# AleoNet/snarkVM

Measured on AMD Instinct MI355X. Metric: BLS12-377 G1 MSM scalar-point pairs/sec (+ Fr NTT elements/sec in ntt_*), higher is better.
Workload: dtype u32 limbs (29-bit radix) modular integer arithmetic, Fq 377-bit / Fr 253-bit; 1 GPU; G1 Pippenger MSM 2^24 (BASELINE.json configs[1]), bases (i+1)G registered in HBM, uniform scalars in HBM; independent instance per GPU; scalars=uniform, lg_ntt=24, window_bits=auto, base_tables=12, table_bits=22, pipelined_batch=True

## Files before the change

include/snarkvm_hip.h:

```cpp
#ifndef SNARKVM_HIP_H
#define SNARKVM_HIP_H

#include <stddef.h>
#include <stdint.h>

#ifdef __cplusplus
extern "C" {
#endif

typedef struct {
    int32_t code;
    char *message;
} RustError;

enum NTTInputOutputOrder { NN = 0, NR = 1, RN = 2, RR = 3 };
enum NTTDirection { Forward = 0, Inverse = 1 };
enum NTTType { Standard = 0, Coset = 1 };


RustError snarkvm_ntt(void *inout, uint32_t lg_domain_size, enum NTTInputOutputOrder ntt_order,
                      enum NTTDirection ntt_direction, enum NTTType ntt_type);

RustError snarkvm_polymul(void *out, size_t pcount, const void *polynomials, const void *plens, size_t ecount,
                          const void *evaluations, const void *elens, uint32_t lg_domain_size);

RustError snarkvm_msm(void *out, const void *points_with_infinity, size_t npoints, const void *scalars,
                      size_t ffi_affine_sz);
RustError snarkvm_hip_set_base_cache(int tables);
RustError snarkvm_hip_set_base_cache_verified(int tables);
void snarkvm_hip_base_cache_stats(uint64_t *out, int reset);


int snarkvm_hip_device_count(void);
int snarkvm_hip_batch_lanes(size_t npoints);
RustError snarkvm_hip_set_devices(const int32_t *ids, size_t n);
RustError snarkvm_hip_set_device(int device);
int snarkvm_hip_num_devices(void);

RustError snarkvm_hip_malloc(void **d_ptr, size_t bytes, int device);
RustError snarkvm_hip_free(void *d_ptr);
RustError snarkvm_hip_memcpy_h2d(void *d_dst, const void *src, size_t bytes);
RustError snarkvm_hip_memcpy_d2h(void *dst, const void *d_src, size_t bytes);
RustError snarkvm_hip_memcpy_d2d(void *d_dst, const void *d_src, size_t bytes);
RustError snarkvm_hip_memset(void *d_dst, int value, size_t bytes);

RustError snarkvm_hip_ntt_device(void *d_inout, uint32_t lg_domain_size, int ntt_order, int ntt_direction,
                                 int ntt_type);
RustError snarkvm_hip_ntt_device_batch(void *const *d_inouts, size_t count, uint32_t lg_domain_size, int ntt_order,
                                       const int *ntt_directions, const int *ntt_types);

RustError snarkvm_hip_polymul_device(void *d_out, size_t pcount, const void *const *d_polys, const size_t *plens, size_t ecount,
                                     const void *const *d_evals, const size_t *elens, uint32_t lg_domain_size);

RustError snarkvm_hip_scope_begin(const void *d_any);
RustError snarkvm_hip_scope_end(void);
enum { SNARKVM_HIP_SCOPE_ASYNC_MSM = 1, SNARKVM_HIP_SCOPE_STABLE_INPUTS = 2, SNARKVM_HIP_SCOPE_MSM_IN_STREAM = 4 };
RustError snarkvm_hip_scope_begin_ex(const void *d_any, uint32_t flags);
RustError snarkvm_hip_scope_collect(const void *out);
RustError snarkvm_hip_scope_set_flags(uint32_t flags);
void *snarkvm_hip_scope_stream(void);

typedef struct snarkvm_hip_bases snarkvm_hip_bases_t;
RustError snarkvm_hip_register_bases(snarkvm_hip_bases_t **handle, const void *points, size_t npoints,
                                     size_t ffi_affine_sz, int on_device);
RustError snarkvm_hip_register_bases_tables(snarkvm_hip_bases_t **handle, const void *points, size_t npoints,
                                            size_t ffi_affine_sz, int on_device, int tables);
RustError snarkvm_hip_register_bases_windowed(snarkvm_hip_bases_t **handle, const void *points, size_t npoints,
                                              size_t ffi_affine_sz, int on_device, int tables, int window_bits);
void snarkvm_hip_free_bases(snarkvm_hip_bases_t *handle);

RustError snarkvm_hip_register_bases_serialized(snarkvm_hip_bases_t **handle, const void *bytes, size_t npoints,
                                                int compressed, int validate, int tables);
RustError snarkvm_hip_g1_deserialize(void *out_affine, const void *bytes, size_t n, int compressed, int validate);
RustError snarkvm_hip_g1_serialize(void *out_bytes, const void *affine, size_t n, size_t ffi_affine_sz, int compressed);

RustError snarkvm_hip_g2_deserialize(void *out_affine, const void *bytes, size_t n, int validate);
RustError snarkvm_hip_g2_serialize(void *out_bytes, const void *affine, size_t n, size_t ffi_affine_sz);
RustError snarkvm_hip_g2_deserialize_compressed(void *out_affine, const void *bytes, size_t n, int validate);
RustError snarkvm_hip_g2_serialize_compressed(void *out_bytes, const void *affine, size_t n, size_t ffi_affine_sz);

RustError snarkvm_hip_msm_registered(void *out, const snarkvm_hip_bases_t *handle, size_t offset, size_t npoints,
                                     const void *scalars, int scalars_on_device, int window_bits);

RustError snarkvm_hip_msm_registered_ex(void *out, const snarkvm_hip_bases_t *handle, size_t off0, size_t n0,
                                        size_t off1, size_t n1, const void *scalars, int scalars_on_device,
                                        int scalars_montgomery, int window_bits);

RustError snarkvm_hip_msm_registered_batch(void *outs, const snarkvm_hip_bases_t *handle, size_t count,
                                           const size_t *offsets, const size_t *npoints, const void *const *scalars,
                                           int scalars_on_device, int scalars_montgomery, int window_bits);

RustError snarkvm_hip_msm_registered_batch_ex(void *outs, const snarkvm_hip_bases_t *handle, size_t count, const size_t *off0,
                                              const size_t *n0, const size_t *off1, const size_t *n1,
                                              const void *const *scalars, int scalars_on_device, int scalars_montgomery,
                                              int window_bits);

RustError snarkvm_hip_g1_sum(void *out, const void *in_projective, size_t n);

RustError snarkvm_hip_g1_to_affine(void *out_affine, const void *in_projective, size_t n);

RustError snarkvm_hip_msm_g2(void *out, const void *points_with_infinity, size_t npoints, const void *scalars,
                             size_t ffi_affine_sz);

typedef struct snarkvm_hip_bases_g2 snarkvm_hip_bases_g2_t;
RustError snarkvm_hip_register_bases_g2(snarkvm_hip_bases_g2_t **handle, const void *points, size_t npoints,
                                        size_t ffi_affine_sz, int tables, int window_bits);
void snarkvm_hip_free_bases_g2(snarkvm_hip_bases_g2_t *handle);
RustError snarkvm_hip_msm_g2_registered(void *out, const snarkvm_hip_bases_g2_t *handle, size_t offset, size_t npoints,
                                        const void *scalars, int scalars_on_device, int window_bits);
RustError snarkvm_hip_msm_g2_registered_batch(void *outs, const snarkvm_hip_bases_g2_t *handle, size_t count,
                                              const size_t *offsets, const size_t *npoints, const void *const *scalars,
                                              int scalars_on_device, int window_bits);

RustError snarkvm_hip_g1_fixed_base_msm(void *out_projective, const void *g_affine, const void *scalars, size_t n);
RustError snarkvm_hip_g1_group_ntt(void *inout_projective, uint32_t lg_domain_size, int inverse);

RustError snarkvm_hip_fr_mul_device(void *d_out, const void *d_a, const void *d_b, size_t n);
RustError snarkvm_hip_fr_convert_device(void *d_out, const void *d_in, size_t n, int to_bigint);

RustError snarkvm_hip_fr_vec_op(int op, void *out, const void *a, const void *b, const void *c, const void *scalar,
                                size_t n, int on_device);
RustError snarkvm_hip_fr_divide_by_linear(void *quotient, void *remainder, const void *poly, size_t n,
                                          const void *point, int on_device);
RustError snarkvm_hip_fr_batch_inversion_and_mul(void *inout, size_t n, const void *coeff, int on_device);
RustError snarkvm_hip_fr_distribute_powers(void *inout, size_t n, const void *g, const void *c, int on_device);
RustError snarkvm_hip_fr_lagrange_coefficients(void *out, uint32_t lg_domain_size, const void *tau, int on_device);
RustError snarkvm_hip_fr_divide_by_vanishing(void *quotient, void *remainder, const void *poly, size_t len,
                                             size_t domain_size, int on_device);
RustError snarkvm_hip_fr_mul_by_vanishing(void *out, const void *poly, size_t len, size_t domain_size, int on_device);

RustError snarkvm_hip_fr_lincomb(void *out, size_t n_out, size_t count, const void *const *polys, const size_t *lens, const void *coeffs,
                                 int on_device);

enum { SNARKVM_HIP_FR_REDUCE_SUM = 0, SNARKVM_HIP_FR_REDUCE_DOT = 1 };
RustError snarkvm_hip_fr_reduce(int op, void *result, const void *a, const void *b, size_t n, int on_device);
RustError snarkvm_hip_fr_reduce_strided(int op, void *results, const void *a, const void *b, size_t n, size_t count, size_t stride,
                                        int b_shared);
RustError snarkvm_hip_fr_support(uint64_t *out3, const void *v, size_t n, int on_device);
RustError snarkvm_hip_fr_support_strided(uint64_t *out, const void *v, size_t n, size_t count, size_t stride);

typedef struct snarkvm_hip_fr_matrix snarkvm_hip_fr_matrix_t;
RustError snarkvm_hip_fr_matrix_register(snarkvm_hip_fr_matrix_t **handle, size_t rows, size_t cols, const uint64_t *row_ptr, const uint32_t *col_idx,
                                         const void *vals);
void snarkvm_hip_fr_matrix_free(snarkvm_hip_fr_matrix_t *handle);
RustError snarkvm_hip_fr_spmv(void *y, size_t n_out, const snarkvm_hip_fr_matrix_t *handle, const void *x, size_t count, size_t stride_x, size_t stride_y,
                              int on_device);

RustError snarkvm_hip_fr_vec_op_strided(int op, void *out, const void *a, const void *b, const void *c, const void *scalar,
                                        size_t n, size_t count, size_t stride);
RustError snarkvm_hip_fr_divide_by_linear_strided(void *quotients, void *remainders, const void *polys, size_t n,
                                                  const void *point, size_t count, size_t stride);
RustError snarkvm_hip_fr_divide_by_vanishing_strided(void *quotients, void *remainders, const void *polys, size_t len,
// ... 47 lines not shown
```

rust/snarkvm-algorithms-hip/src/sys.rs:

```rust
#![allow(non_camel_case_types, non_snake_case, clippy::too_many_arguments, clippy::missing_safety_doc)]
use super::{Error, NTTDirection, NTTInputOutputOrder, NTTType};
use core::ffi::{c_char, c_void};

#[repr(C)]
pub struct snarkvm_hip_bases_t {
    _private: [u8; 0],
}
#[repr(C)]
pub struct snarkvm_hip_bases_g2_t {
    _private: [u8; 0],
}
#[repr(C)]
pub struct snarkvm_hip_fr_matrix_t {
    _private: [u8; 0],
}

pub const SNARKVM_HIP_SCOPE_ASYNC_MSM: u32 = 1;
pub const SNARKVM_HIP_SCOPE_STABLE_INPUTS: u32 = 2;
pub const SNARKVM_HIP_SCOPE_MSM_IN_STREAM: u32 = 4;
pub const SNARKVM_HIP_FR_REDUCE_SUM: u32 = 0;
pub const SNARKVM_HIP_FR_REDUCE_DOT: u32 = 1;

extern "C" {
    pub fn snarkvm_ntt(inout: *mut c_void, lg_domain_size: u32, ntt_order: NTTInputOutputOrder, ntt_direction: NTTDirection, ntt_type: NTTType) -> Error;
    pub fn snarkvm_polymul(out: *mut c_void, pcount: usize, polynomials: *const c_void, plens: *const c_void, ecount: usize, evaluations: *const c_void, elens: *const c_void, lg_domain_size: u32) -> Error;
    pub fn snarkvm_msm(out: *mut c_void, points_with_infinity: *const c_void, npoints: usize, scalars: *const c_void, ffi_affine_sz: usize) -> Error;
    pub fn snarkvm_hip_set_base_cache(tables: i32) -> Error;
    pub fn snarkvm_hip_set_base_cache_verified(tables: i32) -> Error;
    pub fn snarkvm_hip_base_cache_stats(out: *mut u64, reset: i32);
    pub fn snarkvm_hip_device_count() -> i32;
    pub fn snarkvm_hip_batch_lanes(npoints: usize) -> i32;
    pub fn snarkvm_hip_set_devices(ids: *const i32, n: usize) -> Error;
    pub fn snarkvm_hip_set_device(device: i32) -> Error;
    pub fn snarkvm_hip_num_devices() -> i32;
    pub fn snarkvm_hip_malloc(d_ptr: *mut *mut c_void, bytes: usize, device: i32) -> Error;
    pub fn snarkvm_hip_free(d_ptr: *mut c_void) -> Error;
    pub fn snarkvm_hip_memcpy_h2d(d_dst: *mut c_void, src: *const c_void, bytes: usize) -> Error;
    pub fn snarkvm_hip_memcpy_d2h(dst: *mut c_void, d_src: *const c_void, bytes: usize) -> Error;
    pub fn snarkvm_hip_memcpy_d2d(d_dst: *mut c_void, d_src: *const c_void, bytes: usize) -> Error;
    pub fn snarkvm_hip_memset(d_dst: *mut c_void, value: i32, bytes: usize) -> Error;
    pub fn snarkvm_hip_ntt_device(d_inout: *mut c_void, lg_domain_size: u32, ntt_order: i32, ntt_direction: i32, ntt_type: i32) -> Error;
    pub fn snarkvm_hip_ntt_device_batch(d_inouts: *const *mut c_void, count: usize, lg_domain_size: u32, ntt_order: i32, ntt_directions: *const i32, ntt_types: *const i32) -> Error;
    pub fn snarkvm_hip_polymul_device(d_out: *mut c_void, pcount: usize, d_polys: *const *const c_void, plens: *const usize, ecount: usize, d_evals: *const *const c_void, elens: *const usize, lg_domain_size: u32) -> Error;
    pub fn snarkvm_hip_scope_begin(d_any: *const c_void) -> Error;
    pub fn snarkvm_hip_scope_end() -> Error;
    pub fn snarkvm_hip_scope_begin_ex(d_any: *const c_void, flags: u32) -> Error;
    pub fn snarkvm_hip_scope_collect(out: *const c_void) -> Error;
    pub fn snarkvm_hip_scope_set_flags(flags: u32) -> Error;
    pub fn snarkvm_hip_scope_stream() -> *mut c_void;
    pub fn snarkvm_hip_register_bases(handle: *mut *mut snarkvm_hip_bases_t, points: *const c_void, npoints: usize, ffi_affine_sz: usize, on_device: i32) -> Error;
    pub fn snarkvm_hip_register_bases_tables(handle: *mut *mut snarkvm_hip_bases_t, points: *const c_void, npoints: usize, ffi_affine_sz: usize, on_device: i32, tables: i32) -> Error;
    pub fn snarkvm_hip_register_bases_windowed(handle: *mut *mut snarkvm_hip_bases_t, points: *const c_void, npoints: usize, ffi_affine_sz: usize, on_device: i32, tables: i32, window_bits: i32) -> Error;
    pub fn snarkvm_hip_free_bases(handle: *mut snarkvm_hip_bases_t);
    pub fn snarkvm_hip_register_bases_serialized(handle: *mut *mut snarkvm_hip_bases_t, bytes: *const c_void, npoints: usize, compressed: i32, validate: i32, tables: i32) -> Error;
    pub fn snarkvm_hip_g1_deserialize(out_affine: *mut c_void, bytes: *const c_void, n: usize, compressed: i32, validate: i32) -> Error;
    pub fn snarkvm_hip_g1_serialize(out_bytes: *mut c_void, affine: *const c_void, n: usize, ffi_affine_sz: usize, compressed: i32) -> Error;
    pub fn snarkvm_hip_g2_deserialize(out_affine: *mut c_void, bytes: *const c_void, n: usize, validate: i32) -> Error;
    pub fn snarkvm_hip_g2_serialize(out_bytes: *mut c_void, affine: *const c_void, n: usize, ffi_affine_sz: usize) -> Error;
    pub fn snarkvm_hip_g2_deserialize_compressed(out_affine: *mut c_void, bytes: *const c_void, n: usize, validate: i32) -> Error;
    pub fn snarkvm_hip_g2_serialize_compressed(out_bytes: *mut c_void, affine: *const c_void, n: usize, ffi_affine_sz: usize) -> Error;
    pub fn snarkvm_hip_msm_registered(out: *mut c_void, handle: *const snarkvm_hip_bases_t, offset: usize, npoints: usize, scalars: *const c_void, scalars_on_device: i32, window_bits: i32) -> Error;
    pub fn snarkvm_hip_msm_registered_ex(out: *mut c_void, handle: *const snarkvm_hip_bases_t, off0: usize, n0: usize, off1: usize, n1: usize, scalars: *const c_void, scalars_on_device: i32, scalars_montgomery: i32, window_bits: i32) -> Error;
    pub fn snarkvm_hip_msm_registered_batch(outs: *mut c_void, handle: *const snarkvm_hip_bases_t, count: usize, offsets: *const usize, npoints: *const usize, scalars: *const *const c_void, scalars_on_device: i32, scalars_montgomery: i32, window_bits: i32) -> Error;
    pub fn snarkvm_hip_msm_registered_batch_ex(outs: *mut c_void, handle: *const snarkvm_hip_bases_t, count: usize, off0: *const usize, n0: *const usize, off1: *const usize, n1: *const usize, scalars: *const *const c_void, scalars_on_device: i32, scalars_montgomery: i32, window_bits: i32) -> Error;
    pub fn snarkvm_hip_g1_sum(out: *mut c_void, in_projective: *const c_void, n: usize) -> Error;
    pub fn snarkvm_hip_g1_to_affine(out_affine: *mut c_void, in_projective: *const c_void, n: usize) -> Error;
    pub fn snarkvm_hip_msm_g2(out: *mut c_void, points_with_infinity: *const c_void, npoints: usize, scalars: *const c_void, ffi_affine_sz: usize) -> Error;
    pub fn snarkvm_hip_register_bases_g2(handle: *mut *mut snarkvm_hip_bases_g2_t, points: *const c_void, npoints: usize, ffi_affine_sz: usize, tables: i32, window_bits: i32) -> Error;
    pub fn snarkvm_hip_free_bases_g2(handle: *mut snarkvm_hip_bases_g2_t);
    pub fn snarkvm_hip_msm_g2_registered(out: *mut c_void, handle: *const snarkvm_hip_bases_g2_t, offset: usize, npoints: usize, scalars: *const c_void, scalars_on_device: i32, window_bits: i32) -> Error;
    pub fn snarkvm_hip_msm_g2_registered_batch(outs: *mut c_void, handle: *const snarkvm_hip_bases_g2_t, count: usize, offsets: *const usize, npoints: *const usize, scalars: *const *const c_void, scalars_on_device: i32, window_bits: i32) -> Error;
    pub fn snarkvm_hip_g1_fixed_base_msm(out_projective: *mut c_void, g_affine: *const c_void, scalars: *const c_void, n: usize) -> Error;
    pub fn snarkvm_hip_g1_group_ntt(inout_projective: *mut c_void, lg_domain_size: u32, inverse: i32) -> Error;
    pub fn snarkvm_hip_fr_mul_device(d_out: *mut c_void, d_a: *const c_void, d_b: *const c_void, n: usize) -> Error;
    pub fn snarkvm_hip_fr_convert_device(d_out: *mut c_void, d_in: *const c_void, n: usize, to_bigint: i32) -> Error;
    pub fn snarkvm_hip_fr_vec_op(op: i32, out: *mut c_void, a: *const c_void, b: *const c_void, c: *const c_void, scalar: *const c_void, n: usize, on_device: i32) -> Error;
    pub fn snarkvm_hip_fr_divide_by_linear(quotient: *mut c_void, remainder: *mut c_void, poly: *const c_void, n: usize, point: *const c_void, on_device: i32) -> Error;
    pub fn snarkvm_hip_fr_batch_inversion_and_mul(inout: *mut c_void, n: usize, coeff: *const c_void, on_device: i32) -> Error;
    pub fn snarkvm_hip_fr_distribute_powers(inout: *mut c_void, n: usize, g: *const c_void, c: *const c_void, on_device: i32) -> Error;
    pub fn snarkvm_hip_fr_lagrange_coefficients(out: *mut c_void, lg_domain_size: u32, tau: *const c_void, on_device: i32) -> Error;
    pub fn snarkvm_hip_fr_divide_by_vanishing(quotient: *mut c_void, remainder: *mut c_void, poly: *const c_void, len: usize, domain_size: usize, on_device: i32) -> Error;
    pub fn snarkvm_hip_fr_mul_by_vanishing(out: *mut c_void, poly: *const c_void, len: usize, domain_size: usize, on_device: i32) -> Error;
    pub fn snarkvm_hip_fr_lincomb(out: *mut c_void, n_out: usize, count: usize, polys: *const *const c_void, lens: *const usize, coeffs: *const c_void, on_device: i32) -> Error;
    pub fn snarkvm_hip_fr_reduce(op: i32, result: *mut c_void, a: *const c_void, b: *const c_void, n: usize, on_device: i32) -> Error;
    pub fn snarkvm_hip_fr_reduce_strided(op: i32, results: *mut c_void, a: *const c_void, b: *const c_void, n: usize, count: usize, stride: usize, b_shared: i32) -> Error;
    pub fn snarkvm_hip_fr_support(out3: *mut u64, v: *const c_void, n: usize, on_device: i32) -> Error;
    pub fn snarkvm_hip_fr_support_strided(out: *mut u64, v: *const c_void, n: usize, count: usize, stride: usize) -> Error;
    pub fn snarkvm_hip_fr_matrix_register(handle: *mut *mut snarkvm_hip_fr_matrix_t, rows: usize, cols: usize, row_ptr: *const u64, col_idx: *const u32, vals: *const c_void) -> Error;
    pub fn snarkvm_hip_fr_matrix_free(handle: *mut snarkvm_hip_fr_matrix_t);
    pub fn snarkvm_hip_fr_spmv(y: *mut c_void, n_out: usize, handle: *const snarkvm_hip_fr_matrix_t, x: *const c_void, count: usize, stride_x: usize, stride_y: usize, on_device: i32) -> Error;
    pub fn snarkvm_hip_fr_vec_op_strided(op: i32, out: *mut c_void, a: *const c_void, b: *const c_void, c: *const c_void, scalar: *const c_void, n: usize, count: usize, stride: usize) -> Error;
    pub fn snarkvm_hip_fr_divide_by_linear_strided(quotients: *mut c_void, remainders: *mut c_void, polys: *const c_void, n: usize, point: *const c_void, count: usize, stride: usize) -> Error;
    pub fn snarkvm_hip_fr_divide_by_vanishing_strided(quotients: *mut c_void, remainders: *mut c_void, polys: *const c_void, len: usize, domain_size: usize, count: usize, stride: usize) -> Error;
    pub fn snarkvm_hip_g1_generate_bases_device(d_out: *mut c_void, start: u64, npoints: usize) -> Error;
    pub fn snarkvm_hip_set_profiling(enabled: i32);
    pub fn snarkvm_hip_get_phase_count() -> i32;
    pub fn snarkvm_hip_get_phase_name(i: i32) -> *const c_char;
    pub fn snarkvm_hip_get_phase_ms(i: i32) -> f64;
    pub fn snarkvm_hip_coalescer_stats(out: *mut u64, reset: i32);
    pub fn snarkvm_hip_alloc_stats(out: *mut u64, reset: i32);
    pub fn snarkvm_hip_synchronize() -> Error;
    pub fn snarkvm_hip_selftest_field(field: i32, op: i32, a: *const c_void, b: *const c_void, out: *mut c_void, n: usize) -> i32;
    pub fn snarkvm_hip_selftest_g1_msm_naive(points_with_infinity: *const c_void, npoints: usize, ffi_affine_sz: usize, scalars: *const c_void, out: *mut c_void) -> i32;
    pub fn snarkvm_hip_selftest_msm_plan(n: usize, window_bits: i32, tables: i32, table_bits: i32, out: *mut u32) -> i32;
    pub fn snarkvm_hip_selftest_g1_finish(planes_projective: *const c_void, pos: *const i32, n: usize, out: *mut c_void) -> i32;
    pub fn snarkvm_hip_selftest_fq_lazy(seed: u64, iters: i32) -> i32;
    pub fn snarkvm_hip_selftest_g1_lazy_tail(seed: u64, iters: i32) -> i32;
    pub fn snarkvm_hip_selftest_fq2_pair(points: *const c_void, npoints: usize, seed: u64, iters: i32) -> i32;
    pub fn snarkvm_hip_selftest_g2_hex(points: *const c_void, npoints: usize, seed: u64, iters: i32) -> i32;
    pub fn snarkvm_hip_devtest_g2_tail_repeat(points: *const c_void, npoints: usize, m: i32, hb: i32, threads: i32, plane_threads: i32, hex: i32, quads: i32, iters: i32, report: *mut u32) -> Error;
    pub fn snarkvm_hip_selftest_ntt_plan(lg: u32, out: *mut i32) -> i32;
    pub fn snarkvm_hip_selftest_ntt_twiddle(kind: i32, lg: u32, pass: i32, inverse: i32, x: *const u64, n: usize, out: *mut c_void) -> i32;
    pub fn snarkvm_hip_selftest_ntt_index(lg: u32, plan: *const i32, npass: i32) -> i32;
    pub fn snarkvm_hip_selftest_ntt_host(inout: *mut c_void, lg: u32, plan: *const i32, npass: i32, dir: i32, type_: i32) -> i32;
    pub fn snarkvm_hip_selftest_fr_lincomb(out: *mut c_void, n_out: usize, count: usize, polys: *const *const c_void, lens: *const usize, coeffs: *const c_void) -> i32;
    pub fn snarkvm_hip_selftest_fr_reduce(op: i32, out: *mut c_void, a: *const c_void, b: *const c_void, n: usize, blocks: u32, threads: u32) -> i32;
    pub fn snarkvm_hip_selftest_fr_support(out3: *mut u64, v: *const c_void, n: usize, blocks: u32, threads: u32) -> i32;
    pub fn snarkvm_hip_selftest_fr_reduce_geometry(n: usize, out4: *mut u32) -> i32;
    pub fn snarkvm_hip_selftest_fr_spmv(y: *mut c_void, n_out: usize, rows: usize, cols: usize, row_ptr: *const u64, col_idx: *const u32, vals: *const c_void, x: *const c_void, seg: u32, width: u32) -> i32;
    pub fn snarkvm_hip_selftest_fr_spmv_geometry(rows: usize, nnz: usize, out4: *mut u32) -> i32;
    pub fn snarkvm_hip_devtest_field(field: i32, op: i32, a: *const c_void, b: *const c_void, out: *mut c_void, n: usize) -> Error;
    pub fn snarkvm_hip_selftest_field_ext(op: i32, in_: *const c_void, out: *mut c_void, n: usize) -> i32;
    pub fn snarkvm_hip_devtest_field_ext(op: i32, in_: *const c_void, out: *mut c_void, n: usize) -> Error;
}
```

snarkvm_amd/_lib.py:

```python
import ctypes
import os

_HERE = os.path.dirname(os.path.abspath(__file__))
LIB_PATH = os.environ.get("SNARKVM_HIP_LIB") or os.path.join(_HERE, "lib", "libsnarkvm_hip.so")

SYMBOLS = [
    "snarkvm_ntt", "snarkvm_polymul", "snarkvm_msm", "snarkvm_hip_set_base_cache", "snarkvm_hip_set_base_cache_verified", "snarkvm_hip_base_cache_stats",
    "snarkvm_hip_device_count", "snarkvm_hip_batch_lanes", "snarkvm_hip_set_device", "snarkvm_hip_set_devices", "snarkvm_hip_num_devices",
    "snarkvm_hip_malloc", "snarkvm_hip_free", "snarkvm_hip_memcpy_h2d", "snarkvm_hip_memcpy_d2h", "snarkvm_hip_memcpy_d2d", "snarkvm_hip_memset", "snarkvm_hip_ntt_device", "snarkvm_hip_ntt_device_batch", "snarkvm_hip_polymul_device",
    "snarkvm_hip_scope_begin", "snarkvm_hip_scope_end", "snarkvm_hip_scope_begin_ex", "snarkvm_hip_scope_collect", "snarkvm_hip_scope_set_flags", "snarkvm_hip_scope_stream", "snarkvm_hip_alloc_stats",
    "snarkvm_hip_register_bases", "snarkvm_hip_register_bases_tables", "snarkvm_hip_register_bases_windowed", "snarkvm_hip_free_bases", "snarkvm_hip_msm_registered", "snarkvm_hip_msm_g2",
    "snarkvm_hip_msm_registered_ex", "snarkvm_hip_msm_registered_batch", "snarkvm_hip_msm_registered_batch_ex", "snarkvm_hip_g1_to_affine",
    "snarkvm_hip_fr_mul_device", "snarkvm_hip_fr_convert_device", "snarkvm_hip_g1_generate_bases_device",
    "snarkvm_hip_fr_vec_op", "snarkvm_hip_fr_divide_by_linear", "snarkvm_hip_fr_batch_inversion_and_mul",
    "snarkvm_hip_fr_distribute_powers", "snarkvm_hip_fr_lagrange_coefficients", "snarkvm_hip_fr_divide_by_vanishing",
    "snarkvm_hip_fr_mul_by_vanishing", "snarkvm_hip_fr_lincomb",
    "snarkvm_hip_fr_reduce", "snarkvm_hip_fr_reduce_strided", "snarkvm_hip_fr_support", "snarkvm_hip_fr_support_strided",
    "snarkvm_hip_fr_matrix_register", "snarkvm_hip_fr_matrix_free", "snarkvm_hip_fr_spmv",
    "snarkvm_hip_fr_vec_op_strided", "snarkvm_hip_fr_divide_by_linear_strided", "snarkvm_hip_fr_divide_by_vanishing_strided",
    "snarkvm_hip_register_bases_serialized", "snarkvm_hip_g1_deserialize", "snarkvm_hip_g1_serialize", "snarkvm_hip_g1_sum", "snarkvm_hip_g2_deserialize", "snarkvm_hip_g2_serialize", "snarkvm_hip_g2_deserialize_compressed", "snarkvm_hip_g2_serialize_compressed",
    "snarkvm_hip_register_bases_g2", "snarkvm_hip_free_bases_g2", "snarkvm_hip_msm_g2_registered", "snarkvm_hip_msm_g2_registered_batch",
    "snarkvm_hip_g1_fixed_base_msm", "snarkvm_hip_g1_group_ntt",
    "snarkvm_hip_set_profiling", "snarkvm_hip_get_phase_count", "snarkvm_hip_get_phase_name",
    "snarkvm_hip_get_phase_ms", "snarkvm_hip_synchronize", "snarkvm_hip_coalescer_stats",
    "snarkvm_hip_selftest_field", "snarkvm_hip_selftest_g1_msm_naive", "snarkvm_hip_selftest_msm_plan", "snarkvm_hip_selftest_g1_finish", "snarkvm_hip_selftest_fq_lazy", "snarkvm_hip_selftest_g1_lazy_tail", "snarkvm_hip_selftest_ntt_plan", "snarkvm_hip_selftest_ntt_twiddle", "snarkvm_hip_selftest_ntt_index", "snarkvm_hip_selftest_ntt_host", "snarkvm_hip_selftest_fq2_pair", "snarkvm_hip_selftest_g2_hex", "snarkvm_hip_selftest_fr_lincomb", "snarkvm_hip_selftest_fr_reduce", "snarkvm_hip_selftest_fr_support", "snarkvm_hip_selftest_fr_reduce_geometry", "snarkvm_hip_selftest_fr_spmv", "snarkvm_hip_selftest_fr_spmv_geometry", "snarkvm_hip_devtest_field", "snarkvm_hip_devtest_g2_tail_repeat", "snarkvm_hip_selftest_field_ext", "snarkvm_hip_devtest_field_ext",
]


class RustError(ctypes.Structure):
    _fields_ = [("code", ctypes.c_int32), ("message", ctypes.c_void_p)]


class HipError(RuntimeError):
    def __init__(self, code, message):
        super().__init__(f"snarkvm_hip error {code}: {message}")
        self.code = code
        self.message = message


_lib = None
_libc = None


def lib():
    global _lib, _libc
    if _lib is None:
        if not os.path.exists(LIB_PATH):
            raise ImportError(
                f"{LIB_PATH} is missing - build it with `python -m snarkvm_amd.build` (hipcc, gfx950). "
                "snarkvm_amd has no CPU fallback.")
        if not os.environ.get("SNARKVM_HIP_NO_TORCH"):
            try:
                import torch
            except ImportError:
                pass
        L = ctypes.CDLL(LIB_PATH)
        err_fns = ["snarkvm_ntt", "snarkvm_polymul", "snarkvm_msm", "snarkvm_hip_set_base_cache", "snarkvm_hip_set_base_cache_verified", "snarkvm_hip_set_device", "snarkvm_hip_set_devices",
                   "snarkvm_hip_malloc", "snarkvm_hip_free", "snarkvm_hip_memcpy_h2d", "snarkvm_hip_memcpy_d2h", "snarkvm_hip_memcpy_d2d", "snarkvm_hip_memset", "snarkvm_hip_ntt_device", "snarkvm_hip_ntt_device_batch", "snarkvm_hip_polymul_device",
                   "snarkvm_hip_scope_begin", "snarkvm_hip_scope_end", "snarkvm_hip_scope_begin_ex", "snarkvm_hip_scope_collect", "snarkvm_hip_scope_set_flags",
                   "snarkvm_hip_register_bases", "snarkvm_hip_register_bases_tables", "snarkvm_hip_register_bases_windowed", "snarkvm_hip_msm_registered", "snarkvm_hip_msm_g2", "snarkvm_hip_msm_registered_ex", "snarkvm_hip_msm_registered_batch", "snarkvm_hip_msm_registered_batch_ex", "snarkvm_hip_g1_to_affine", "snarkvm_hip_fr_mul_device",
                   "snarkvm_hip_fr_convert_device", "snarkvm_hip_g1_generate_bases_device", "snarkvm_hip_synchronize",
                   "snarkvm_hip_fr_vec_op", "snarkvm_hip_fr_divide_by_linear", "snarkvm_hip_fr_batch_inversion_and_mul", "snarkvm_hip_fr_distribute_powers", "snarkvm_hip_fr_lagrange_coefficients", "snarkvm_hip_fr_divide_by_vanishing", "snarkvm_hip_fr_mul_by_vanishing", "snarkvm_hip_fr_lincomb",
                   "snarkvm_hip_fr_reduce", "snarkvm_hip_fr_reduce_strided", "snarkvm_hip_fr_support", "snarkvm_hip_fr_support_strided",
                   "snarkvm_hip_fr_matrix_register", "snarkvm_hip_fr_spmv",
                   "snarkvm_hip_fr_vec_op_strided", "snarkvm_hip_fr_divide_by_linear_strided", "snarkvm_hip_fr_divide_by_vanishing_strided",
                   "snarkvm_hip_register_bases_serialized", "snarkvm_hip_g1_deserialize", "snarkvm_hip_g1_serialize", "snarkvm_hip_g1_sum", "snarkvm_hip_g2_deserialize", "snarkvm_hip_g2_serialize", "snarkvm_hip_g2_deserialize_compressed", "snarkvm_hip_g2_serialize_compressed",
                   "snarkvm_hip_register_bases_g2", "snarkvm_hip_msm_g2_registered", "snarkvm_hip_msm_g2_registered_batch",
                   "snarkvm_hip_g1_fixed_base_msm", "snarkvm_hip_g1_group_ntt",
                   "snarkvm_hip_devtest_field", "snarkvm_hip_devtest_g2_tail_repeat", "snarkvm_hip_devtest_field_ext"]
        for name in err_fns:
            getattr(L, name).restype = RustError
        L.snarkvm_hip_device_count.restype = ctypes.c_int
        L.snarkvm_hip_batch_lanes.restype = ctypes.c_int
        L.snarkvm_hip_num_devices.restype = ctypes.c_int
        L.snarkvm_hip_selftest_g1_finish.restype = ctypes.c_int
        L.snarkvm_hip_selftest_fq_lazy.restype = ctypes.c_int
        L.snarkvm_hip_selftest_g1_lazy_tail.restype = ctypes.c_int
        for name in ("snarkvm_hip_selftest_ntt_plan", "snarkvm_hip_selftest_ntt_twiddle", "snarkvm_hip_selftest_ntt_index", "snarkvm_hip_selftest_ntt_host"):
            getattr(L, name).restype = ctypes.c_int
        L.snarkvm_hip_selftest_fq2_pair.restype = ctypes.c_int
        L.snarkvm_hip_selftest_g2_hex.restype = ctypes.c_int
        L.snarkvm_hip_selftest_fr_lincomb.restype = ctypes.c_int
        L.snarkvm_hip_get_phase_count.restype = ctypes.c_int
        L.snarkvm_hip_get_phase_name.restype = ctypes.c_char_p
        L.snarkvm_hip_get_phase_ms.restype = ctypes.c_double
        L.snarkvm_hip_selftest_field.restype = ctypes.c_int
        L.snarkvm_hip_selftest_field_ext.restype = ctypes.c_int
        L.snarkvm_hip_selftest_field_ext.argtypes = [ctypes.c_int, ctypes.c_void_p, ctypes.c_void_p, ctypes.c_size_t]
        L.snarkvm_hip_devtest_field_ext.argtypes = L.snarkvm_hip_selftest_field_ext.argtypes
        L.snarkvm_hip_selftest_g1_msm_naive.restype = ctypes.c_int
        L.snarkvm_hip_selftest_msm_plan.restype = ctypes.c_int
        L.snarkvm_hip_free_bases.restype = None
        L.snarkvm_hip_free_bases_g2.restype = None
        L.snarkvm_hip_set_profiling.restype = None
        L.snarkvm_hip_coalescer_stats.restype = None
        L.snarkvm_hip_base_cache_stats.restype = None
        L.snarkvm_hip_alloc_stats.restype = None
        L.snarkvm_hip_scope_stream.restype = ctypes.c_void_p
        L.snarkvm_hip_scope_begin_ex.argtypes = [ctypes.c_void_p, ctypes.c_uint32]
        L.snarkvm_hip_scope_set_flags.argtypes = [ctypes.c_uint32]
        L.snarkvm_hip_alloc_stats.argtypes = [ctypes.c_void_p, ctypes.c_int]
        L.snarkvm_hip_coalescer_stats.argtypes = [ctypes.c_void_p, ctypes.c_int]
        L.snarkvm_hip_base_cache_stats.argtypes = [ctypes.c_void_p, ctypes.c_int]
        L.snarkvm_hip_malloc.argtypes = [ctypes.POINTER(ctypes.c_void_p), ctypes.c_size_t, ctypes.c_int]
        L.snarkvm_hip_free.argtypes = [ctypes.c_void_p]
        L.snarkvm_hip_memcpy_h2d.argtypes = [ctypes.c_void_p, ctypes.c_void_p, ctypes.c_size_t]
        L.snarkvm_hip_memcpy_d2h.argtypes = [ctypes.c_void_p, ctypes.c_void_p, ctypes.c_size_t]
        L.snarkvm_hip_memcpy_d2d.argtypes = [ctypes.c_void_p, ctypes.c_void_p, ctypes.c_size_t]
        L.snarkvm_hip_memset.argtypes = [ctypes.c_void_p, ctypes.c_int, ctypes.c_size_t]
        L.snarkvm_hip_polymul_device.argtypes = [ctypes.c_void_p, ctypes.c_size_t, ctypes.POINTER(ctypes.c_void_p), ctypes.POINTER(ctypes.c_size_t),
                                                 ctypes.c_size_t, ctypes.POINTER(ctypes.c_void_p), ctypes.POINTER(ctypes.c_size_t), ctypes.c_uint32]
        L.snarkvm_hip_fr_lincomb.argtypes = [ctypes.c_void_p, ctypes.c_size_t, ctypes.c_size_t, ctypes.POINTER(ctypes.c_void_p), ctypes.POINTER(ctypes.c_size_t),
                                             ctypes.c_void_p, ctypes.c_int]
        L.snarkvm_hip_selftest_fr_lincomb.argtypes = L.snarkvm_hip_fr_lincomb.argtypes[:-1]
        L.snarkvm_hip_fr_reduce.argtypes = [ctypes.c_int, ctypes.c_void_p, ctypes.c_void_p, ctypes.c_void_p, ctypes.c_size_t, ctypes.c_int]
        L.snarkvm_hip_fr_reduce_strided.argtypes = [ctypes.c_int, ctypes.c_void_p, ctypes.c_void_p, ctypes.c_void_p, ctypes.c_size_t, ctypes.c_size_t, ctypes.c_size_t, ctypes.c_int]
        L.snarkvm_hip_fr_support.argtypes = [ctypes.c_void_p, ctypes.c_void_p, ctypes.c_size_t, ctypes.c_int]
        L.snarkvm_hip_fr_support_strided.argtypes = [ctypes.c_void_p, ctypes.c_void_p, ctypes.c_size_t, ctypes.c_size_t, ctypes.c_size_t]
        L.snarkvm_hip_selftest_fr_reduce.argtypes = [ctypes.c_int, ctypes.c_void_p, ctypes.c_void_p, ctypes.c_void_p, ctypes.c_size_t, ctypes.c_uint32, ctypes.c_uint32]
        L.snarkvm_hip_selftest_fr_support.argtypes = [ctypes.c_void_p, ctypes.c_void_p, ctypes.c_size_t, ctypes.c_uint32, ctypes.c_uint32]
        L.snarkvm_hip_selftest_fr_reduce_geometry.argtypes = [ctypes.c_size_t, ctypes.c_void_p]
        for name in ("snarkvm_hip_selftest_fr_reduce", "snarkvm_hip_selftest_fr_support", "snarkvm_hip_selftest_fr_reduce_geometry"):
            getattr(L, name).restype = ctypes.c_int
        L.snarkvm_hip_fr_matrix_register.argtypes = [ctypes.POINTER(ctypes.c_void_p), ctypes.c_size_t, ctypes.c_size_t, ctypes.c_void_p, ctypes.c_void_p, ctypes.c_void_p]
        L.snarkvm_hip_fr_matrix_free.argtypes = [ctypes.c_void_p]
        L.snarkvm_hip_fr_matrix_free.restype = None
        L.snarkvm_hip_fr_spmv.argtypes = [ctypes.c_void_p, ctypes.c_size_t, ctypes.c_void_p, ctypes.c_void_p, ctypes.c_size_t, ctypes.c_size_t, ctypes.c_size_t, ctypes.c_int]
        L.snarkvm_hip_selftest_fr_spmv.argtypes = [ctypes.c_void_p, ctypes.c_size_t, ctypes.c_size_t, ctypes.c_size_t, ctypes.c_void_p, ctypes.c_void_p, ctypes.c_void_p, ctypes.c_void_p,
                                                   ctypes.c_uint32, ctypes.c_uint32]
        L.snarkvm_hip_selftest_fr_spmv_geometry.argtypes = [ctypes.c_size_t, ctypes.c_size_t, ctypes.c_void_p]
        L.snarkvm_hip_selftest_fr_spmv.restype = ctypes.c_int
        L.snarkvm_hip_selftest_fr_spmv_geometry.restype = ctypes.c_int
        _libc = ctypes.CDLL(None)
        _libc.free.argtypes = [ctypes.c_void_p]
        _lib = L
    return _lib


def check(err):
    if err.code != 0:
        msg = ctypes.string_at(err.message).decode(errors="replace") if err.message else ""
        if err.message:
            _libc.free(err.message)
        raise HipError(err.code, msg)


def device_count():
    return lib().snarkvm_hip_device_count()
```

snarkvm_amd/csrc/api.hip:

```cpp
#define SV_TU_G1
#include "runtime.hip.h"
#include "ffl.hip.h"

runtime_t g_rt;
thread_local thread_scope_t g_tl_scope;
thread_scope_t::~thread_scope_t() {
    if (!lane) return;
    pending.clear();
    (void)hipStreamSynchronize(lane->stream);
    for (int i = 0; i < naux; i++) {
        (void)hipStreamSynchronize(aux[i]->stream);
        aux[i]->dev->give(aux[i], true);
    }
    lane->in_scope = false;
    lane->deferred.clear();
    lane->deferred_bytes = 0;
    if (!lane->tw_leases.empty()) ntt_tw_release(lane->dev, lane->tw_leases);
    lane->dev->give(lane, true);
    lane = nullptr;
}
std::atomic<uint64_t> g_co_stats[4];
static std::atomic<uint64_t> g_alloc_stats[5];
void sv_alloc_note(int slot, size_t bytes, double ms) {
    g_alloc_stats[slot].fetch_add(1, std::memory_order_relaxed);
    g_alloc_stats[slot + 1].fetch_add(bytes, std::memory_order_relaxed);
    g_alloc_stats[4].fetch_add((uint64_t)(ms * 1e3), std::memory_order_relaxed);
}

struct tl_free_list_t {
    std::vector<void*> v;
    ~tl_free_list_t() {
        for (void* p : v) (void)hipFree(p);
    }
};
static thread_local tl_free_list_t g_tl_free;
void sv_defer_free(void* p) { g_tl_free.v.push_back(p); }
void sv_drain_frees() {
    if (g_tl_free.v.empty()) return;
    std::vector<void*> mine;
    mine.swap(g_tl_free.v);
    for (void* p : mine) (void)hipFree(p);
}

extern "C" {

int snarkvm_hip_device_count(void) {
    int n = 0;
    if (hipGetDeviceCount(&n) != hipSuccess) return 0;
    return n;
}
int snarkvm_hip_batch_lanes(size_t npoints) { return batch_lanes(npoints); }
RustError snarkvm_hip_set_devices(const int32_t* ids, size_t n) {
    std::lock_guard<std::mutex> lk(g_rt.cfg_mu);
    if (n == 0 || !ids) return fail(1, "snarkvm_hip_set_devices: empty device list");
    std::vector<int> v(ids, ids + n);
    if (g_rt.configured) {
        bool same = v.size() == g_rt.devs.size();
        for (size_t i = 0; same && i < v.size(); i++) same = g_rt.devs[i]->physical == v[i];
        if (!same) return fail(1, "snarkvm_hip_set_devices: the runtime is already initialised on another device set");
        return ok();
    }
    g_rt.want = v;
    return ok();
}
RustError snarkvm_hip_set_device(int device) {
    const int32_t d = device;
    return snarkvm_hip_set_devices(&d, 1);
}
int snarkvm_hip_num_devices(void) {
    try {
        return g_rt.ndev();
    } catch (...) {
        return 0;
    }
}
void snarkvm_hip_set_profiling(int enabled) { g_rt.profiling.store(enabled != 0); }
int snarkvm_hip_get_phase_count(void) {
    std::lock_guard<std::mutex> lk(g_rt.prof_mu);
    return (int)g_rt.last_phases.size();
}
const char* snarkvm_hip_get_phase_name(int i) {
    std::lock_guard<std::mutex> lk(g_rt.prof_mu);
    return (i >= 0 && i < (int)g_rt.last_phases.size()) ? g_rt.last_phases[i].first.c_str() : "";
}
double snarkvm_hip_get_phase_ms(int i) {
    std::lock_guard<std::mutex> lk(g_rt.prof_mu);
    return (i >= 0 && i < (int)g_rt.last_phases.size()) ? g_rt.last_phases[i].second : 0.0;
// ... 92 lines not shown
}

static constexpr uint32_t SCOPE_FLAGS_ALL = SNARKVM_HIP_SCOPE_ASYNC_MSM | SNARKVM_HIP_SCOPE_STABLE_INPUTS | SNARKVM_HIP_SCOPE_MSM_IN_STREAM;
RustError snarkvm_hip_scope_begin_ex(const void* d_any, uint32_t flags) {
    API_TRY
    thread_scope_t& sc = tl_scope();
    if (sc.lane) throw hip_failure{hipErrorInvalidValue, "scope_begin: the calling thread already has an open scope", __LINE__};
    if (flags & ~SCOPE_FLAGS_ALL) throw hip_failure{hipErrorInvalidValue, "scope_begin: unknown flag", __LINE__};
    g_rt.configure();
    const int nd = (int)g_rt.devs.size();
    int dev = device_for(d_any, d_any ? 1 : 0);
    if (dev < 0) dev = (int)(g_rt.rr.fetch_add(1) % (uint32_t)nd);
    device_t* d = g_rt.devs[dev].get();
    int prev = -1;
    if (hipGetDevice(&prev) != hipSuccess) prev = 0;
    lane_t* l = d->take_for_scope(true);
    try {
        HIP_TRY(hipSetDevice(d->physical));
        d->init();
        tu_kernel_attributes(d->logical);
    } catch (...) {
        d->give(l, true);
        (void)hipSetDevice(prev);
        throw;
    }
    l->begin_call();
    l->in_scope = true;
    l->pin_used = 0;
    l->scope_events_used = 0;
    sc = thread_scope_t();
    sc.lane = l;
    sc.prev_device = prev;
    sc.flags = flags;
    API_CATCH
}
RustError snarkvm_hip_scope_begin(const void* d_any) { return snarkvm_hip_scope_begin_ex(d_any, 0); }
void* snarkvm_hip_scope_stream(void) {
    lane_t* l = tl_scope().lane;
    return l ? (void*)l->stream : nullptr;
}
RustError snarkvm_hip_scope_set_flags(uint32_t flags) {
    API_TRY
    thread_scope_t& sc = tl_scope();
    if (!sc.lane) throw hip_failure{hipErrorInvalidValue, "scope_set_flags: the calling thread has no open scope", __LINE__};
    if (flags & ~SCOPE_FLAGS_ALL) throw hip_failure{hipErrorInvalidValue, "scope_set_flags: unknown flag", __LINE__};
    sc.flags = flags;
    API_CATCH
}
RustError snarkvm_hip_scope_collect(const void* out) {
    API_TRY
    scope_collect(out);
    API_CATCH
}
RustError snarkvm_hip_scope_end(void) {
    thread_scope_t& sc = tl_scope();
    lane_t* l = sc.lane;
    if (!l) return ok();
    RustError r = ok();
    try {
        scope_flush();
    } catch (const hip_failure& f) {
        r = from_failure(f);
    } catch (const std::exception& e) {
        r = fail(1, std::string("snarkvm_hip: scope_end: ") + e.what());
    } catch (...) {
        r = fail(1, "snarkvm_hip: scope_end failed");
    }
    l->in_scope = false;
    l->deferred.clear();
    l->deferred_bytes = 0;
    for (int i = 0; i < sc.naux; i++) {
        (void)hipStreamSynchronize(sc.aux[i]->stream);
        sc.aux[i]->dev->give(sc.aux[i], true);
    }
    const int prev = sc.prev_device;
    sc = thread_scope_t();
    l->dev->give(l, true);
    if (prev >= 0) (void)hipSetDevice(prev);
    return r;
}

static void precompute_tables(lane_t& c, snarkvm_hip_bases* h, g1_aff_mem_t* d) { precompute_tables_run<fq_t>(c, d, h->n, h->tables, h->table_bits); }
static void register_bases_impl(snarkvm_hip_bases_t** handle, const void* points, size_t npoints, size_t ffi_affine_sz, int on_device, int tables,
                                int table_bits) {
    if (!handle) throw hip_failure{hipErrorInvalidValue, "register_bases: null handle", __LINE__};
    if (npoints && !points) throw hip_failure{hipErrorInvalidValue, "register_bases: null points", __LINE__};
    if (ffi_affine_sz < 104 || (ffi_affine_sz & 7)) throw hip_failure{hipErrorInvalidValue, "register_bases: bad stride", __LINE__};
    check_tables(tables, table_bits, "register_bases");
    scope_flush();
    const int nd = g_rt.ndev();
    std::unique_ptr<snarkvm_hip_bases> h(new snarkvm_hip_bases());
    h->n = npoints;
    h->tables = tables;
    h->table_bits = table_bits ? table_bits : 256 / tables;
    h->d.assign(nd, nullptr);
    const size_t bytes = (size_t)tables * npoints * sizeof(g1_aff_mem_t);
    try {
        if (npoints) {
            const int owner = on_device ? device_for(points, 1) : -1;
            auto build = [&](int dev) {
                lane_guard lg(dev);
                lane_t& c = lg.c();
                HIP_TRY(hipMalloc((void**)&h->d[dev], bytes));
                const uint8_t* src = (const uint8_t*)points;
                if (!on_device) {
                    c.bases_tmp.ensure(npoints * ffi_affine_sz);
                    HIP_TRY(hipMemcpyAsync(c.bases_tmp.p, points, npoints * ffi_affine_sz, hipMemcpyHostToDevice, c.stream));
                    src = c.bases_tmp.as<uint8_t>();
                }
                convert_bases<fq_t>(c, src, ffi_affine_sz, npoints, h->d[dev]);
                precompute_tables(c, h.get(), h->d[dev]);
                bases_to_lazy_form(c, h->d[dev], (size_t)tables * npoints);
                HIP_TRY(hipStreamSynchronize(c.stream));
            };
            std::vector<int> all;
            for (int d = 0; d < nd; d++) all.push_back(d);
            if (!on_device) {
                for_each_device(all, build);
            } else {
                build(owner);
                for (int d = 0; d < nd; d++) {
                    if (d == owner) continue;
                    lane_guard lg(d);
                    HIP_TRY(hipMalloc((void**)&h->d[d], bytes));
                    HIP_TRY(hipMemcpyPeerAsync(h->d[d], g_rt.devs[d]->physical, h->d[owner], g_rt.devs[owner]->physical, bytes, lg.c().stream));
                    HIP_TRY(hipStreamSynchronize(lg.c().stream));
                }
            }
        }
    } catch (...) {
        h->free_all();
        throw;
    }
    *handle = h.release();
}
RustError snarkvm_hip_register_bases(snarkvm_hip_bases_t** handle, const void* points, size_t npoints, size_t ffi_affine_sz, int on_device) {
    API_TRY
    register_bases_impl(handle, points, npoints, ffi_affine_sz, on_device, 1, 0);
    API_CATCH
}
RustError snarkvm_hip_register_bases_tables(snarkvm_hip_bases_t** handle, const void* points, size_t npoints, size_t ffi_affine_sz, int on_device,
                                            int tables) {
    API_TRY
    register_bases_impl(handle, points, npoints, ffi_affine_sz, on_device, tables, 0);
    API_CATCH
}
RustError snarkvm_hip_register_bases_windowed(snarkvm_hip_bases_t** handle, const void* points, size_t npoints, size_t ffi_affine_sz, int on_device,
                                              int tables, int window_bits) {
    API_TRY
    if (window_bits <= 0) throw hip_failure{hipErrorInvalidValue, "register_bases_windowed: window_bits must be positive", __LINE__};
    register_bases_impl(handle, points, npoints, ffi_affine_sz, on_device, tables, window_bits);
    API_CATCH
}
void snarkvm_hip_free_bases(snarkvm_hip_bases_t* h) {
    if (!h) return;
    h->free_all();
    delete h;
}
}
snarkvm_hip_bases* sv_new_bases_handle(size_t npoints, int tables, int table_bits) {
    snarkvm_hip_bases* h = new snarkvm_hip_bases();
    h->n = npoints;
    h->tables = tables;
    h->table_bits = table_bits;
    h->d.assign(g_rt.ndev(), nullptr);
    return h;
}
void sv_precompute_tables(lane_t& c, snarkvm_hip_bases* h, g1_aff_mem_t* d) { precompute_tables(c, h, d); }
extern "C" {

static void check_window_bits(int window_bits, const char* who) {
    if (window_bits && (window_bits < 2 || window_bits > MSM_C_MAX)) throw std::runtime_error(std::string(who) + ": window_bits must be 0 or 2..23");
}
static void msm_registered_host_scalars(void* out, const snarkvm_hip_bases* h, size_t off0, size_t n0, size_t off1, size_t n1, const void* scalars,
                                        int scalars_montgomery, int window_bits) {
    const size_t n = n0 + n1;
    scope_flush();
    const int nd = g_rt.ndev();
    static const int trace = getenv("SNARKVM_HIP_TRACE") ? atoi(getenv("SNARKVM_HIP_TRACE")) : 0;
    const double t_begin = host_now_ms();
    size_t parts = n / MSM_SPLIT_MIN;
    if (parts > (size_t)nd) parts = (size_t)nd;
    if (parts < 1) parts = 1;
    const size_t chunk = msm_scalar_chunk_pairs();
    if (n >= 2 * chunk && (n + chunk - 1) / chunk > parts) parts = (n + chunk - 1) / chunk;
    std::vector<size_t> bound;
    const int geo = tuning().scalar_geo;
    if (nd == 1 && geo > 1 && tuning().taper != 0 && n >= ((size_t)1 << 22)) {
        parts = n >= ((size_t)1 << 23) ? 3 : 2;
        size_t wsum = 0, w = 1;
        for (size_t i = 0; i < parts; i++, w *= (size_t)geo) wsum += w;
        size_t acc_w = 0;
        w = 1;
        bound.push_back(0);
        for (size_t i = 0; i < parts; i++, w *= (size_t)geo) {
            acc_w += w;
            bound.push_back(i + 1 == parts ? n : (size_t)((unsigned __int128)n * acc_w / wsum));
        }
    } else {
        for (size_t i = 0; i <= parts; i++) bound.push_back(n * i / parts);
    }
    const int ndu = (int)(parts < (size_t)nd ? parts : (size_t)nd);
    std::unique_ptr<msm_accum_t<fq_t>> acc(new msm_accum_t<fq_t>());
    std::mutex acc_mu;
    std::vector<int> devs;
    if (ndu == 1) {
        devs.push_back(-1);
    } else {
        for (int d = 0; d < ndu; d++) devs.push_back(d);
    }
    const size_t slot = msm_plane_bytes<fq_t>();
    for_each_device(devs, [&](int dev) {
        std::vector<size_t> mine;
        for (size_t i = (dev < 0 ? 0 : (size_t)dev); i < parts; i += (size_t)ndu) mine.push_back(i);
        lane_guard lg;
        lg.acquire(dev, mine.size() > 2 ? 3 : (int)mine.size());
        const size_t L = lg.lanes.size();
        size_t max_cnt = 0;
        for (size_t j = 0; j < mine.size(); j++) {
            const size_t cnt = bound[mine[j] + 1] - bound[mine[j]];
            max_cnt = cnt > max_cnt ? cnt : max_cnt;
        }
        const bool use_sink = tuning().taper != 0 && mine.size() >= 2;
        std::vector<msm_pending_t> pend(use_sink ? 1 : mine.size());
        int chunk_c = window_bits;
        msm_bucket_sink_t sink;
        std::vector<hipEvent_t> merged;
        for (size_t l = 0; l < L; l++) {
            lane_t& c = *lg.lanes[l];
            c.begin_call();
            c.scalars_tmp.ensure(max_cnt * 32 + 32);
            c.pin.ensure(slot * (use_sink ? 1 : (mine.size() + L - 1) / L));
        }
        if (use_sink) {
            lane_t& c0 = *lg.lanes[0];
            const msm_plan_t pl = msm_make_plan(max_cnt, window_bits, h->tables, h->table_bits);
            chunk_c = pl.c;
            sink.nbt = (uint32_t)pl.W * pl.nb;
            sink.L = 1;
            const size_t bytes = (size_t)sink.nbt * msm_partial_bytes<fq_t>();
            c0.sink_acc.ensure(bytes);
            sink.acc = c0.sink_acc.p;
            HIP_TRY(hipMemsetAsync(sink.acc, 0, bytes, c0.stream));
            hipEvent_t ready = c0.new_event();
            HIP_TRY(hipEventRecord(ready, c0.stream));
            for (size_t l = 1; l < L; l++) HIP_TRY(hipStreamWaitEvent(lg.lanes[l]->stream, ready, 0));
            for (size_t j = 0; j < mine.size(); j++) merged.push_back(lg.lanes[j % L]->new_event());
        }
        auto upload = [&](size_t j, hipStream_t st) {
            lane_t& c = *lg.lanes[j % L];
            const size_t lo = bound[mine[j]], hi = bound[mine[j] + 1];
// ... 271 lines not shown
    for (size_t k = k0; k <= k1; k++)
        if (memcmp(&e.samples[k * 97], e.host + k * CACHE_STEP * e.stride, 97) != 0) return false;
    return true;
}
static void base_cache_remember(const uint8_t* p, size_t npoints, size_t stride, bool verified) {
    for (size_t i = g_base_cache.size(); i-- > 0;)
        if (g_base_cache[i].stride == stride && g_base_cache[i].host >= p && g_base_cache[i].host + g_base_cache[i].n * stride <= p + npoints * stride)
            base_cache_drop(i);
    while (g_base_cache.size() >= CACHE_MAX) {
        size_t lru = 0;
        for (size_t i = 1; i < g_base_cache.size(); i++)
            if (g_base_cache[i].last_use < g_base_cache[lru].last_use) lru = i;
        base_cache_drop(lru);
    }
    base_cache_entry e;
    e.host = p;
    e.n = npoints;
    e.stride = stride;
    e.verified = verified;
    if (!verified)
        for (size_t k = 0; k * CACHE_STEP < e.n; k++) e.samples.insert(e.samples.end(), e.host + k * CACHE_STEP * e.stride, e.host + k * CACHE_STEP * e.stride + 97);
    e.last_use = ++g_cache_tick;
    g_base_cache.push_back(std::move(e));
}
struct base_cache_use {
    std::shared_ptr<snarkvm_hip_bases> h;
    std::shared_ptr<const host_shadow_t> shadow;
    size_t offset = 0;
};
static base_cache_use base_cache_lookup(const void* points, size_t npoints, size_t stride) {
    base_cache_use u;
    const bool verified = base_cache_verified();
    std::lock_guard<std::mutex> lk(g_cache_mu);
    g_bc_stats[0]++;
    for (size_t i = g_base_cache.size(); i-- > 0;)
        if (g_base_cache[i].verified != verified) base_cache_drop(i);
    const uint8_t* p = (const uint8_t*)points;
    for (size_t i = 0; i < g_base_cache.size(); i++) {
        if (g_base_cache[i].stride != stride || p < g_base_cache[i].host || p + npoints * stride > g_base_cache[i].host + g_base_cache[i].n * stride ||
            (size_t)(p - g_base_cache[i].host) % stride)
            continue;
        const size_t off = (size_t)(p - g_base_cache[i].host) / stride;
        if (!verified && !samples_match(g_base_cache[i], off, npoints)) {
            base_cache_drop(i);
            break;
        }
        g_base_cache[i].last_use = ++g_cache_tick;
        if (!g_base_cache[i].h) {
            if (g_base_cache[i].failed || off != 0 || npoints != g_base_cache[i].n) return u;
            int tables = base_cache_tables(), bits = 0;
            if (tables == 16 && g_base_cache[i].n >= ((size_t)1 << 24)) tables = 12, bits = 22;
            else if (tables == 16 && g_base_cache[i].n >= ((size_t)1 << 21)) tables = 13, bits = 20;
            else if (tables == 16 && g_base_cache[i].n < ((size_t)1 << 18)) tables = 17, bits = 15;
            const size_t need = (size_t)tables * g_base_cache[i].n * sizeof(g1_aff_mem_t), need_host = verified ? npoints * PAYLOAD : 0;
            if (need > base_cache_cap() || need_host > base_cache_host_cap()) return u;
            for (;;) {
                size_t used = 0, used_host = 0, lru = (size_t)-1;
                for (size_t j = 0; j < g_base_cache.size(); j++) {
                    used += g_base_cache[j].bytes();
                    used_host += g_base_cache[j].host_bytes();
                    if (j != i && g_base_cache[j].h && (lru == (size_t)-1 || g_base_cache[j].last_use < g_base_cache[lru].last_use)) lru = j;
                }
                if ((used + need <= base_cache_cap() && used_host + need_host <= base_cache_host_cap()) || lru == (size_t)-1) break;
                base_cache_drop(lru);
                if (lru < i) i--;
            }
            std::shared_ptr<host_shadow_t> shadow;
            snarkvm_hip_bases_t* nh = nullptr;
            try {
                if (verified) {
                    shadow = std::make_shared<host_shadow_t>();
                    shadow->b.reset(new uint8_t[npoints * PAYLOAD]);
                    shadow->n = npoints;
                    auto job = std::make_shared<host_job_t>();
                    job->nchunks = (npoints + VERIFY_CHUNK - 1) / VERIFY_CHUNK;
                    uint8_t* dst = shadow->b.get();
                    job->fn = [p, dst, npoints, stride](host_job_t&, size_t k) {
                        const size_t lo = k * VERIFY_CHUNK, hi = lo + VERIFY_CHUNK < npoints ? lo + VERIFY_CHUNK : npoints;
                        for (size_t j = lo; j < hi; j++) memcpy(dst + j * PAYLOAD, p + j * stride, PAYLOAD);
                    };
                    verify_pool().submit(job);
                    job->wait();
                }
                register_bases_impl(&nh, points, npoints, stride, 0, tables, bits);
            } catch (...) {
                (void)hipGetLastError();
                g_base_cache[i].failed = true;
                return u;
            }
            g_base_cache[i].h = std::shared_ptr<snarkvm_hip_bases>(nh, [](snarkvm_hip_bases* b) { snarkvm_hip_free_bases(b); });
            g_base_cache[i].shadow = shadow;
            g_bc_stats[2]++;
        } else if (verified) {
            u.shadow = g_base_cache[i].shadow;
        } else {
            g_bc_stats[1]++;
        }
        u.offset = off;
        u.h = g_base_cache[i].h;
        return u;
    }
    base_cache_remember(p, npoints, stride, verified);
    return u;
}

static void msm_cached_verified(void* out, const base_cache_use& u, const void* points, size_t npoints, const void* scalars, size_t stride) {
    auto job = std::make_shared<host_job_t>();
    job->nchunks = (npoints + VERIFY_CHUNK - 1) / VERIFY_CHUNK;
    const uint8_t* host = (const uint8_t*)points;
    const std::shared_ptr<const host_shadow_t> keep = u.shadow;
    const size_t off = u.offset;
    job->fn = [host, keep, off, npoints, stride](host_job_t& j, size_t k) {
        if (j.flag.load(std::memory_order_relaxed)) return;
        const size_t lo = k * VERIFY_CHUNK, cnt = lo + VERIFY_CHUNK < npoints ? VERIFY_CHUNK : npoints - lo;
        if (payload_equal(host + lo * stride, stride, keep->b.get() + (off + lo) * PAYLOAD, cnt))
            j.bytes.fetch_add(cnt * PAYLOAD, std::memory_order_relaxed);
        else
            j.flag.store(true, std::memory_order_relaxed);
    };
    verify_pool().submit(job);
    alignas(16) uint8_t res[144];
    try {
        if (msm_coalescible(*u.h, npoints, 0))
            msm_single_coalesced(res, u.h.get(), u.offset, npoints, 0, 0, scalars, 0, 0, 0);
        else
            msm_registered_host_scalars(res, u.h.get(), u.offset, npoints, 0, 0, scalars, 0, 0);
    } catch (...) {
        job->flag.store(true);
        job->wait();
        throw;
    }
    const double t_ready = host_now_ms();
    job->wait();
    g_bc_stats[5] += (uint64_t)((host_now_ms() - t_ready) * 1e3);
    g_bc_stats[4] += job->bytes.load();
    if (!job->flag.load()) {
        memcpy(out, res, 144);
        g_bc_stats[1]++;
        return;
    }
    g_bc_stats[3]++;
    {
        std::lock_guard<std::mutex> lk(g_cache_mu);
        for (size_t i = 0; i < g_base_cache.size(); i++)
            if (g_base_cache[i].h == u.h) {
                base_cache_drop(i);
                break;
            }
        if (base_cache_verified()) base_cache_remember(host, npoints, stride, true);
    }
    msm_host_chunked<fq_t>(out, points, npoints, scalars, stride);
}

static RustError base_cache_set(int tables, bool verified, const char* who) {
    if (!(tables == 0 || tables == 1 || tables == 2 || tables == 4 || tables == 8 || tables == 16))
        return fail(1, std::string(who) + ": tables must be 0, 1, 2, 4, 8 or 16");
    const bool was_verified = base_cache_verified();
    g_base_cache_override.store(tables | (verified && tables ? CACHE_VERIFIED : 0), std::memory_order_relaxed);
    if (tables == 0 || was_verified != base_cache_verified()) {
        std::vector<base_cache_entry> drop;
        {
            std::lock_guard<std::mutex> lk(g_cache_mu);
            drop.swap(g_base_cache);
        }
    }
    return ok();
}
// ... 325 lines not shown
```

snarkvm_amd/csrc/api_serde.hip:

```cpp
#include "runtime.hip.h"

snarkvm_hip_bases* sv_new_bases_handle(size_t npoints, int tables, int table_bits);
void sv_precompute_tables(lane_t& c, snarkvm_hip_bases* h, g1_aff_mem_t* d);

static uint32_t g1_deserialize_run(lane_t& c, const void* bytes, size_t n, int compressed, int validate, g1_aff_mem_t* d_native, uint8_t* d_rust) {
    const size_t psz = compressed ? 48 : 96;
    c.bases_tmp.ensure(n * psz);
    c.serde_status.ensure(4);
    HIP_TRY(hipMemcpyAsync(c.bases_tmp.p, bytes, n * psz, hipMemcpyHostToDevice, c.stream));
    HIP_TRY(hipMemsetAsync(c.serde_status.p, 0, 4, c.stream));
    hipLaunchKernelGGL(g1_deserialize_kernel, dim3((unsigned)((n + 63) / 64)), dim3(64), 0, c.stream, c.bases_tmp.as<uint8_t>(), n, compressed, validate,
                       d_native, d_rust, c.serde_status.as<uint32_t>());
    HIP_TRY(hipGetLastError());
    uint32_t st = 0;
    HIP_TRY(hipMemcpyAsync(&st, c.serde_status.p, 4, hipMemcpyDeviceToHost, c.stream));
    HIP_TRY(hipStreamSynchronize(c.stream));
    return st;
}

extern "C" {

RustError snarkvm_hip_register_bases_serialized(snarkvm_hip_bases_t** handle, const void* bytes, size_t npoints, int compressed, int validate,
                                                int tables) {
    API_TRY
    if (!handle || (npoints && !bytes)) throw hip_failure{hipErrorInvalidValue, "register_bases_serialized: null argument", __LINE__};
    check_tables(tables, 0, "register_bases_serialized");
    std::unique_ptr<snarkvm_hip_bases> h(sv_new_bases_handle(npoints, tables, 256 / tables));
    if (npoints) {
        try {
            std::vector<int> all;
            for (int d = 0; d < g_rt.ndev(); d++) all.push_back(d);
            for_each_device(all, [&](int dev) {
                lane_guard lg(dev);
                lane_t& c = lg.c();
                HIP_TRY(hipMalloc((void**)&h->d[dev], (size_t)tables * npoints * sizeof(g1_aff_mem_t)));
                serde_throw_on_status(g1_deserialize_run(c, bytes, npoints, compressed, validate, h->d[dev], nullptr), "register_bases_serialized");
                sv_precompute_tables(c, h.get(), h->d[dev]);
                bases_to_lazy_form(c, h->d[dev], (size_t)tables * npoints);
                HIP_TRY(hipStreamSynchronize(c.stream));
            });
        } catch (...) {
            h->free_all();
            throw;
        }
    }
    *handle = h.release();
    API_CATCH
}
RustError snarkvm_hip_g1_deserialize(void* out_affine, const void* bytes, size_t n, int compressed, int validate) {
    API_BEGIN
    if (n) {
        if (!out_affine || !bytes) throw hip_failure{hipErrorInvalidValue, "g1_deserialize: null argument", __LINE__};
        c.poly[0].ensure(n * 104);
        const uint32_t st = g1_deserialize_run(c, bytes, n, compressed, validate, nullptr, c.poly[0].as<uint8_t>());
        serde_throw_on_status(st, "g1_deserialize");
        HIP_TRY(hipMemcpyAsync(out_affine, c.poly[0].p, n * 104, hipMemcpyDeviceToHost, c.stream));
        HIP_TRY(hipStreamSynchronize(c.stream));
    }
    API_END
}
RustError snarkvm_hip_g1_serialize(void* out_bytes, const void* affine, size_t n, size_t ffi_affine_sz, int compressed) {
    API_BEGIN
    if (n) {
        if (!out_bytes || !affine) throw hip_failure{hipErrorInvalidValue, "g1_serialize: null argument", __LINE__};
        if (ffi_affine_sz < 104 || (ffi_affine_sz & 7)) throw hip_failure{hipErrorInvalidValue, "g1_serialize: bad stride", __LINE__};
        const size_t psz = compressed ? 48 : 96;
        c.bases_tmp.ensure(n * ffi_affine_sz);
        c.poly[0].ensure(n * psz);
        HIP_TRY(hipMemcpyAsync(c.bases_tmp.p, affine, n * ffi_affine_sz, hipMemcpyHostToDevice, c.stream));
        hipLaunchKernelGGL(g1_serialize_kernel, dim3((unsigned)((n + 63) / 64)), dim3(64), 0, c.stream, c.bases_tmp.as<uint8_t>(), ffi_affine_sz, n,
                           compressed, c.poly[0].as<uint8_t>());
        HIP_TRY(hipGetLastError());
        HIP_TRY(hipMemcpyAsync(out_bytes, c.poly[0].p, n * psz, hipMemcpyDeviceToHost, c.stream));
        HIP_TRY(hipStreamSynchronize(c.stream));
    }
    API_END
}

}
```

snarkvm_amd/csrc/ffl.hip.h:

```cpp
#pragma once
#include "ec.hip.h"

namespace sv {

struct FqL {
    static constexpr int N = 13;
    static constexpr int STEPS = 14;
    static constexpr int32_t MOD[13] = {0x00000001, 0x08460000, 0x00000021, 0x16ba8860, 0x14800170, 0x1117dd04, 0x0e3c7bcd,
                                        0x1e601ea2, 0x1b1a22d9, 0x03650a49, 0x118ec170, 0x0f8a21d5, 0x1ae3a461};
    static constexpr int32_t K377[13] = {0x1fffffff, 0x17b9ffff, 0x1fffffde, 0x0945779f, 0x0b7ffe8f, 0x0ee822fb, 0x11c38432,
                                         0x019fe15d, 0x04e5dd26, 0x1c9af5b6, 0x0e713e8f, 0x1075de2a, 0x051c5b9e};
    static constexpr int32_t K435[13] = {0x0677f3e3, 0x01fcf72f, 0x05fc93a0, 0x08eb59fe, 0x0c1a6c3f, 0x122b8005, 0x01c7de9b,
                                         0x0b159718, 0x189a8339, 0x07649107, 0x02e4fa41, 0x13571fee, 0x04eba458};
};
struct FqLConv {
    static constexpr uint32_t C406[13] = {0x19eaf730u, 0x171ffffeu, 0x0d714cf8u, 0x044e31d8u, 0x1eb6e262u, 0x0bfad163u, 0x00d46e9cu,
                                          0x10b6ddbfu, 0x13b9cbddu, 0x075782afu, 0x03bd1d8au, 0x1557cab6u, 0x15742a14u};
    static constexpr uint32_t C399[13] = {0x1fb3d5efu, 0x1759ffffu, 0x161ae2aeu, 0x06bd319fu, 0x15cd6eabu, 0x15c6dfc5u, 0x00a7763du,
                                          0x1e5d80e1u, 0x10d7c95fu, 0x04add573u, 0x1c80b321u, 0x02e104bau, 0x10f92f11u};
    static constexpr uint32_t C348[13] = {0, 0, 0, 0, 0, 0, 0, 0, 0, 0, 0, 0, 1};
};

#if defined(__HIP_DEVICE_COMPILE__)
#define SV_OPAQUE_LIMB(x) asm("" : "+v"(x))
// ... 253 lines not shown
        return {x.to_exact(), y.to_exact(), zz.to_exact(), zzz.to_exact()};
    }
    SV_HD void store_raw(g1_lazy_partial_t* p) const {
        uint4* q = (uint4*)p;
        if (inf) {
#pragma unroll
            for (int i = 0; i < 13; i++) q[i] = make_uint4(0, 0, 0, 0);
            return;
        }
        int32_t t[52];
#pragma unroll
        for (int i = 0; i < 13; i++) t[i] = x.v[i], t[13 + i] = y.v[i], t[26 + i] = zz.v[i], t[39 + i] = zzz.v[i];
#pragma unroll
        for (int i = 0; i < 13; i++) q[i] = make_uint4((uint32_t)t[4 * i], (uint32_t)t[4 * i + 1], (uint32_t)t[4 * i + 2], (uint32_t)t[4 * i + 3]);
    }
    SV_HD static g1_xyzz_t exact_from_raw(const g1_lazy_partial_t* p) {
        const uint4* q = (const uint4*)p;
        int32_t t[52];
#pragma unroll
        for (int i = 0; i < 13; i++) {
            const uint4 u = q[i];
            t[4 * i] = (int32_t)u.x, t[4 * i + 1] = (int32_t)u.y, t[4 * i + 2] = (int32_t)u.z, t[4 * i + 3] = (int32_t)u.w;
        }
        fql_t c[4];
#pragma unroll
        for (int k = 0; k < 4; k++)
#pragma unroll
            for (int i = 0; i < 13; i++) c[k].v[i] = t[13 * k + i];
        return {c[0].to_exact(), c[1].to_exact(), c[2].to_exact(), c[3].to_exact()};
    }
    SV_HD static xyzz_lazy_t from_exact(const g1_xyzz_t& p) {
        xyzz_lazy_t r;
        r.inf = p.is_inf();
        if (r.inf) return infinity();
        r.x = fql_t::from_exact(p.x);
        r.y = fql_t::from_exact(p.y);
        r.zz = fql_t::from_exact(p.zz);
        r.zzz = fql_t::from_exact(p.zzz);
        return r;
    }
    SV_HD bool madd(const fql_t& px, const fql_t& py, bool negate) {
        if (inf) {
            x = px;
            y = py.negate_if(negate).normalized();
            zz = zzz = one();
            inf = false;
            return true;
        }
        const fql_t u2 = fql_t::mul(px, zz);
        const fql_t s2 = fql_t::mul(py.negate_if(negate), zzz);
        const fql_t p = u2 - x;
        const fql_t r = s2 - y;
        if ((((uint32_t)p.v[0] + 4u) & fql_t::MASK) <= 5u) return false;
        const fql_t pp = fql_t::sqr(p);
        const fql_t ppp = fql_t::mul(p, pp);
        const fql_t q = fql_t::mul(x, pp);
        const fql_t rr = fql_t::sqr(r);
        fql_t x3;
        {
            int32_t c = 0;
#pragma unroll
            for (int i = 0; i < fql_t::N - 1; i++) {
                const int32_t t = rr.v[i] - ppp.v[i] - 2 * q.v[i] + c;
                x3.v[i] = (int32_t)((uint32_t)t & fql_t::MASK);
                c = t >> 29;
            }
            x3.v[fql_t::N - 1] = rr.v[fql_t::N - 1] - ppp.v[fql_t::N - 1] - 2 * q.v[fql_t::N - 1] + c;
            SV_OPAQUE_13(x3.v);
        }
        y = fql_t::diff_of_products(r, q - x3, y, ppp);
        x = x3;
        zz = fql_t::mul(zz, pp);
        zzz = fql_t::mul(zzz, ppp);
        return true;
    }
    SV_HD static fql_t one() {
        fql_t r;
#pragma unroll
        for (int i = 0; i < fql_t::N; i++) r.v[i] = (int32_t)FqLConv::C406[i];
        return r;
    }
};

struct fqz_t {
    fql_t a;
    struct mem_t {
        uint32_t w[13];
    };
    static constexpr int N = 13;

    SV_HD static fqz_t zero() { return {fql_t::zero()}; }
    SV_HD static fqz_t one() { return {xyzz_lazy_t::one()}; }
    SV_HD static fqz_t load(const mem_t* p) {
        fqz_t r;
#pragma unroll
        for (int i = 0; i < N; i++) r.a.v[i] = (int32_t)p->w[i];
        return r;
    }
    SV_HD void store(mem_t* p) const {
#pragma unroll
        for (int i = 0; i < N; i++) p->w[i] = (uint32_t)a.v[i];
    }
    SV_HD fqz_t operator*(const fqz_t& b) const { return {fql_t::mul(a, b.a)}; }
    SV_HD fqz_t sqr() const { return {fql_t::sqr(a)}; }
    SV_HD fqz_t operator+(const fqz_t& b) const { return {(a + b.a).normalized()}; }
    SV_HD fqz_t operator-(const fqz_t& b) const { return {(a - b.a).normalized()}; }
    SV_HD fqz_t dbl() const { return {(a + a).normalized()}; }
    SV_HD fqz_t neg() const { return {(fql_t::zero() - a).normalized()}; }
    SV_HD static fqz_t diff_of_products(const fqz_t& x, const fqz_t& y, const fqz_t& z, const fqz_t& w) {
        return {fql_t::diff_of_products(x.a, y.a, z.a, w.a)};
    }
    SV_HD fq_t to_exact() const { return a.to_exact(); }
    SV_HD bool is_zero() const {
        int32_t any = 0;
#pragma unroll
        for (int i = 0; i < N; i++) any |= a.v[i];
        if (any == 0) return true;
        if ((((uint32_t)a.v[0] + 8u) & fql_t::MASK) > 16u) return false;
        return a.to_exact().is_zero();
    }
};

}
```

snarkvm_amd/csrc/msm_sort.hip.h:

```cpp
#pragma once
#include "ffl.hip.h"
#include "ffl2.hip.h"
#include "ffl2p.hip.h"
#include "msm.hip.h"

namespace sv {

static constexpr int SORT_TILE = 8192;
static constexpr int SORT_THREADS = 256;

struct msm_inst_t {
    const uint4* scalars;
    uint32_t n;
    uint32_t n0;
    uint32_t off0, off1;
    uint32_t pstart;
    uint32_t ptiles;
};
struct msm_radix_params_t {
    size_t n;
    int c, W, J;
    int HB, LB;
    uint32_t nb;
    uint32_t tiles_per_row;
// ... 693 lines not shown
            raw = raw_next;
            if (pos + 1 < hi) {
                e_next = sorted[pos + 1];
                raw_next = *slot_of(e_next);
            }
        } else {
            raw = *slot_of(e);
            if (pos + 1 < hi) e_next = sorted[pos + 1];
        }
        acc.add_affine(load_aff<F>(&raw), (e >> 31) != 0);
    }
    store_xyzz<F>(&partial[start_k + part_off], acc);
}

static __global__ void __launch_bounds__(256) g1_partials_to_exact_kernel(const g1_lazy_partial_t* __restrict__ raw, g1_xyzz_mem_t* __restrict__ partial,
                                                                   const uint32_t* __restrict__ start, uint32_t nbt) {
    const uint32_t i = blockIdx.x * blockDim.x + threadIdx.x;
    if (i >= start[nbt]) return;
    g1_store_xyzz(&partial[i], xyzz_lazy_t::exact_from_raw(&raw[i]));
}
static __device__ __noinline__ void lazy_exceptional_add(xyzz_lazy_t* acc, const fql_t* px, const fql_t* py, bool neg) {
    g1_xyzz_t ex = acc->to_exact();
    const fq_t c348 = fq_t::from_table(FqLConv::C348);
    fq_t bx, by;
#pragma unroll
    for (int i = 0; i < 13; i++) bx.v[i] = (uint32_t)px->v[i], by.v[i] = (uint32_t)py->v[i];
    ex.add_affine({bx * c348, by * c348}, neg);
    *acc = xyzz_lazy_t::from_exact(ex);
}
template <bool PREFETCH>
__global__ void __launch_bounds__(256, 1) msm_accumulate_lazy_kernel(const g1_aff_mem_t* __restrict__ bases, const uint32_t* __restrict__ sorted,
                                                              const uint32_t* __restrict__ boff, const uint32_t* __restrict__ start,
                                                              g1_lazy_partial_t* __restrict__ partial, uint32_t nbt, uint32_t S, uint32_t debug_idx_mask) {
    const uint32_t t = blockIdx.x * blockDim.x + threadIdx.x;
    const uint32_t total = boff[nbt];
    const uint64_t lo64 = (uint64_t)t * S;
    if (lo64 >= total) return;
    const uint32_t lo = (uint32_t)lo64;
    const uint32_t hi = (total - lo < S) ? total : lo + S;
    uint32_t k = find_bucket(boff, nbt, lo);
    uint32_t kend = boff[k + 1];
    uint32_t kend2 = boff[k + 2 <= nbt ? k + 2 : nbt];
    uint32_t start_k = start[k];
    uint32_t part_off = t - boff[k] / S;
    xyzz_lazy_t acc = xyzz_lazy_t::infinity();
    auto slot_of = [&](uint32_t e) -> const g1_lazy_slot_t* { return (const g1_lazy_slot_t*)&bases[(e & 0x7fffffffu) & debug_idx_mask]; };
    uint32_t e_cur = sorted[lo];
    uint32_t e_n1 = lo + 1 < hi ? sorted[lo + 1] : 0u;
    g1_lazy_slot_t raw_next = *slot_of(e_cur);
    for (uint32_t pos = lo;; pos++) {
        const bool end = pos >= hi;
        if (end || pos >= kend) {
            acc.store_raw(&partial[start_k + part_off]);
            if (end) break;
            part_off = 0;
            acc.inf = true;
            k++;
            kend = kend2;
            while (pos >= kend) {
                k++;
                kend = boff[k + 1];
            }
            kend2 = boff[k + 2 <= nbt ? k + 2 : nbt];
            start_k = start[k];
        }
        const uint32_t e = e_cur;
        const g1_lazy_slot_t raw = raw_next;
        if (pos + 1 < hi) raw_next = *slot_of(e_n1);
        e_cur = e_n1;
        if (pos + 2 < hi) e_n1 = sorted[pos + 2];
        if (raw.w[26]) continue;
        const bool neg = (e >> 31) != 0;
        fql_t px, py;
        raw.coords(px, py);
        if (!acc.madd(px, py, neg)) {
            xyzz_lazy_t tmp = acc;
            const fql_t tx = px, ty = py;
            lazy_exceptional_add(&tmp, &tx, &ty, neg);
            acc = tmp;
        }
    }
}

static __global__ void __launch_bounds__(256) g2_pair_partials_to_exact_kernel(const g2_pair_partial_t* __restrict__ raw, xyzz_mem_t<fq2_t>* __restrict__ partial,
                                                                        const uint32_t* __restrict__ start, uint32_t nbt) {
    const uint32_t g = blockIdx.x * blockDim.x + threadIdx.x;
    const uint32_t i = g >> 3, k = g & 7;
    if (i >= start[nbt]) return;
    const uint4* q = (const uint4*)&raw[i].w[16 * k];
    uint32_t t[16];
#pragma unroll
    for (int j = 0; j < 4; j++) {
        const uint4 u = q[j];
        t[4 * j] = u.x, t[4 * j + 1] = u.y, t[4 * j + 2] = u.z, t[4 * j + 3] = u.w;
    }
    fql_t c;
#pragma unroll
    for (int j = 0; j < 13; j++) c.v[j] = (int32_t)t[j];
    c.to_exact().store(&((fq_mem_t*)&partial[i])[k]);
}
template <bool PREFETCH>
__global__ void __launch_bounds__(256, 2) msm_accumulate_pair2_kernel(const aff_mem_t<fq2_t>* __restrict__ bases, const uint32_t* __restrict__ sorted,
                                                               const uint32_t* __restrict__ boff, const uint32_t* __restrict__ start,
                                                               g2_pair_partial_t* __restrict__ partial, uint32_t nbt, uint32_t S, uint32_t debug_idx_mask) {
    const uint32_t gt = blockIdx.x * blockDim.x + threadIdx.x;
    const uint32_t t = gt >> 1;
    const int comp = (int)(gt & 1u);
    const uint32_t total = boff[nbt];
    const uint64_t lo64 = (uint64_t)t * S;
    if (lo64 >= total) return;
    const uint32_t lo = (uint32_t)lo64;
    const uint32_t hi = (total - lo < S) ? total : lo + S;
    uint32_t k = find_bucket(boff, nbt, lo);
    uint32_t kend = boff[k + 1];
    uint32_t start_k = start[k];
    uint32_t part_off = t - boff[k] / S;
    fq2p::xyzz_pair_t<fq2p::xp_dev> acc;
    acc.inf = true;
    auto slot_of = [&](uint32_t e) -> const g2_lazy_slot_t* { return (const g2_lazy_slot_t*)&bases[(e & 0x7fffffffu) & debug_idx_mask]; };
    for (uint32_t pos = lo;; pos++) {
        const bool end = pos >= hi;
        if (end || pos >= kend) {
            uint4* q = (uint4*)&partial[start_k + part_off].w[16 * comp];
            if (acc.inf) {
#pragma unroll
                for (int c4 = 0; c4 < 4; c4++)
#pragma unroll
                    for (int j = 0; j < 4; j++) q[8 * c4 + j] = make_uint4(0, 0, 0, 0);
            } else {
                const fql_t* cs[4] = {&acc.x[0], &acc.y[0], &acc.zz[0], &acc.zzz[0]};
#pragma unroll
                for (int c4 = 0; c4 < 4; c4++) {
                    const int32_t* v = cs[c4]->v;
                    q[8 * c4 + 0] = make_uint4((uint32_t)v[0], (uint32_t)v[1], (uint32_t)v[2], (uint32_t)v[3]);
                    q[8 * c4 + 1] = make_uint4((uint32_t)v[4], (uint32_t)v[5], (uint32_t)v[6], (uint32_t)v[7]);
                    q[8 * c4 + 2] = make_uint4((uint32_t)v[8], (uint32_t)v[9], (uint32_t)v[10], (uint32_t)v[11]);
                    q[8 * c4 + 3] = make_uint4((uint32_t)v[12], 0u, 0u, 0u);
                }
            }
            if (end) break;
            part_off = 0;
            acc.inf = true;
            do {
                k++;
                kend = boff[k + 1];
            } while (pos >= kend);
            start_k = start[k];
        }
        const uint32_t e = sorted[pos];
        const g2_lazy_slot_t* sp = slot_of(e);
        if (sp->w[g2_lazy_slot_t::INF_WORD]) continue;
        fql_t px[1], py[1];
        sp->component(comp, px[0], py[0]);
        acc.madd(px, py, (e >> 31) != 0);
    }
}

}
```

snarkvm_amd/csrc/runtime.hip.h:

```cpp
#pragma once
#include <hip/hip_runtime.h>
#include <stdint.h>
#include <stdio.h>
#include <stdlib.h>
#include <string.h>
#include <time.h>

#include <atomic>
#include <chrono>
#include <condition_variable>
#include <deque>
#include <functional>
#include <exception>
#include <memory>
#include <mutex>
#include <stdexcept>
#include <string>
#include <thread>
#include <type_traits>
#include <utility>
#include <vector>

#include "../../include/snarkvm_hip.h"
#include "ec.hip.h"
// ... 272 lines not shown
                return &lane[l];
            }
        }
        return nullptr;
    }
    void give(lane_t* l, bool from_scope = false) {
        {
            std::lock_guard<std::mutex> lk(mu);
            busy &= ~(1u << l->index);
            if (from_scope) scope_held--;
        }
        cv.notify_all();
    }
};

struct runtime_t {
    std::mutex cfg_mu;
    std::vector<int> want;
    std::vector<std::unique_ptr<device_t>> devs;
    bool configured = false;
    std::atomic<uint32_t> rr{0};
    std::atomic<bool> profiling{false};
    std::mutex prof_mu;
    std::vector<std::pair<std::string, double>> last_phases;

    void configure() {
        std::lock_guard<std::mutex> lk(cfg_mu);
        if (configured) return;
        int ndev = 0;
        hipError_t e = hipGetDeviceCount(&ndev);
        if (e != hipSuccess || ndev == 0) throw hip_failure{e == hipSuccess ? hipErrorNoDevice : e, "hipGetDeviceCount (no MI355X visible)", __LINE__};
        std::vector<int> ids = want;
        if (ids.empty()) {
            if (const char* env = getenv("SNARKVM_HIP_DEVICES")) {
                for (const char* p = env; *p;) {
                    char* end = nullptr;
                    long v = strtol(p, &end, 10);
                    if (end == p) break;
                    ids.push_back((int)v);
                    p = (*end == ',') ? end + 1 : end;
                }
            }
        }
        if (ids.empty())
            for (int d = 0; d < ndev; d++) ids.push_back(d);
        for (int id : ids)
            if (id < 0 || id >= ndev) throw hip_failure{hipErrorInvalidDevice, "device index out of range (snarkvm_hip_set_devices / SNARKVM_HIP_DEVICES)", __LINE__};
        for (size_t i = 0; i < ids.size(); i++) {
            devs.emplace_back(new device_t());
            devs.back()->logical = (int)i;
            devs.back()->physical = ids[i];
        }
        configured = true;
    }
    int ndev() {
        configure();
        return (int)devs.size();
    }
    int device_of(const void* ptr) {
        configure();
        hipPointerAttribute_t at;
        if (!ptr || hipPointerGetAttributes(&at, ptr) != hipSuccess) {
            (void)hipGetLastError();
            return -1;
        }
        std::vector<int> match;
        for (auto& d : devs)
            if (d->physical == at.device) match.push_back(d->logical);
        if (match.empty()) return -1;
        return match[rr.fetch_add(1) % match.size()];
    }
};
extern runtime_t g_rt;

static void tu_kernel_attributes(int logical) {
    static std::mutex mu;
    static std::vector<char> done;
    std::lock_guard<std::mutex> lk(mu);
    if ((int)done.size() <= logical) done.resize(logical + 1, 0);
    if (done[logical]) return;
    HIP_TRY(hipFuncSetAttribute((const void*)scan_one_block_kernel, hipFuncAttributeMaxDynamicSharedMemorySize, (int)(SCAN_ONE_MAX * 4)));
#ifdef SV_TU_G1
    HIP_TRY(hipFuncSetAttribute((const void*)msm_accumulate_lazy_kernel<true>, hipFuncAttributeMaxDynamicSharedMemorySize, 128 * 1024));
#endif
#ifdef SV_TU_NTT
    HIP_TRY(hipFuncSetAttribute((const void*)ntt_pass_kernel_v2<false, ntt_arith_u>, hipFuncAttributeMaxDynamicSharedMemorySize, 96 * 1024));
    HIP_TRY(hipFuncSetAttribute((const void*)ntt_pass_kernel_v2<true, ntt_arith_u>, hipFuncAttributeMaxDynamicSharedMemorySize, 96 * 1024));
    HIP_TRY(hipFuncSetAttribute((const void*)ntt_pass_kernel_v2<true, ntt_arith_u, ntt_load_bounded>, hipFuncAttributeMaxDynamicSharedMemorySize, 96 * 1024));
    HIP_TRY(hipFuncSetAttribute((const void*)ntt_pass_kernel_v2<false, ntt_arith_u, ntt_load_product>, hipFuncAttributeMaxDynamicSharedMemorySize, 96 * 1024));
#endif
    done[logical] = 1;
}

static constexpr int SCOPE_AUX_MAX = 7;
struct scope_pending_t {
    hipEvent_t done;
    std::function<void()> finish;
    const void* tag;
};
struct thread_scope_t {
    lane_t* lane = nullptr;
    int prev_device = -1;
    unsigned flags = 0;
    lane_t* aux[SCOPE_AUX_MAX] = {};
    int naux = 0;
    unsigned aux_rr = 0;
    bool aux_exhausted = false;
    std::vector<scope_pending_t> pending;
    thread_scope_t() = default;
    thread_scope_t(const thread_scope_t&) = default;
    thread_scope_t& operator=(const thread_scope_t&) = default;
    ~thread_scope_t();
};
extern thread_local thread_scope_t g_tl_scope;
static thread_scope_t& tl_scope() { return g_tl_scope; }
static void scope_flush() {
    thread_scope_t& sc = tl_scope();
    if (!sc.lane) return;
    std::exception_ptr err;
    for (scope_pending_t& p : sc.pending) {
        try {
            HIP_TRY(hipEventSynchronize(p.done));
            p.finish();
        } catch (...) {
            if (!err) err = std::current_exception();
        }
    }
    sc.pending.clear();
    try {
        sc.lane->flush_scope();
        for (int i = 0; i < sc.naux; i++) HIP_TRY(hipStreamSynchronize(sc.aux[i]->stream));
    } catch (...) {
        if (!err) err = std::current_exception();
    }
    sc.lane->pin_used = 0;
    sc.lane->scope_events_used = 0;
    for (int i = 0; i < sc.naux; i++) sc.aux[i]->pin_used = 0, sc.aux[i]->scope_events_used = 0;
    if (err) std::rethrow_exception(err);
}
static void scope_collect(const void* tag) {
    thread_scope_t& sc = tl_scope();
    if (!sc.lane) return;
    std::exception_ptr err;
    if (tag) {
        auto ready = [](const scope_pending_t& p) {
            const hipError_t e = hipEventQuery(p.done);
            if (e == hipSuccess) return true;
            (void)hipGetLastError();
            return false;
        };
        auto wanted_ready = [&]() {
            for (const scope_pending_t& p : sc.pending)
                if (p.tag == tag && !ready(p)) return false;
            return true;
        };
        for (size_t i = 0; i < sc.pending.size() && !wanted_ready();) {
            if (sc.pending[i].tag != tag && ready(sc.pending[i])) {
                try {
                    sc.pending[i].finish();
                } catch (...) {
                    if (!err) err = std::current_exception();
                }
                sc.pending.erase(sc.pending.begin() + (ptrdiff_t)i);
            } else {
                i++;
            }
// ... 91 lines not shown
        for (size_t i = first_borrowed ? 1 : 0; i < lanes.size(); i++) lanes[i]->dev->give(lanes[i]);
        if (prev_device >= 0) (void)hipSetDevice(prev_device);
    }
};

inline ntt_ctx_t lane_t::ntt_ctx(hipStream_t st) { return ntt_ctx_t{st ? st : stream, &dev->tb, &dev->tw, &tw_leases}; }
inline void lane_t::begin_call() {
    phases.clear();
    events_used = 0;
}
inline void lane_t::phase_begin(const char* name) {
    if (!g_rt.profiling.load(std::memory_order_relaxed)) return;
    phase_rec r{name, new_event(), new_event(), 0.0};
    HIP_TRY(hipEventRecord(r.e0, stream));
    phases.push_back(r);
}
inline void lane_t::phase_end() {
    if (!g_rt.profiling.load(std::memory_order_relaxed) || phases.empty()) return;
    HIP_TRY(hipEventRecord(phases.back().e1, stream));
}
inline void lane_t::phase_host(const char* name, double ms) {
    if (!g_rt.profiling.load(std::memory_order_relaxed)) return;
    phases.push_back(phase_rec{name, nullptr, nullptr, ms});
}
static void ntt_tw_release(device_t* dev, std::vector<void*>& leases) { ntt_tw_release_entries(dev->tw, leases); }
inline void lane_t::flush_scope() {
    HIP_TRY(hipStreamSynchronize(stream));
    for (const deferred_out_t& d : deferred) memcpy(d.dst, pin2.as<uint8_t>() + d.off, d.bytes);
    deferred.clear();
    deferred_bytes = 0;
    if (!tw_leases.empty()) ntt_tw_release(dev, tw_leases);
    sv_drain_frees();
}
inline void lane_t::end_call() {
    if (in_scope) return;
    sv_drain_frees();
    if (!tw_leases.empty()) {
        HIP_TRY(hipStreamSynchronize(stream));
        ntt_tw_release(dev, tw_leases);
    }
    if (phases.empty()) return;
    HIP_TRY(hipStreamSynchronize(stream));
    std::vector<std::pair<std::string, double>> out;
    for (auto& r : phases) {
        if (r.e0) {
            float ms = 0;
            HIP_TRY(hipEventElapsedTime(&ms, r.e0, r.e1));
            r.ms = ms;
        }
        out.emplace_back(r.name, r.ms);
    }
    std::lock_guard<std::mutex> lk(g_rt.prof_mu);
    g_rt.last_phases.swap(out);
}

template <class Fn>
static void for_each_device(const std::vector<int>& devices, Fn fn) {
    if (devices.size() <= 1) {
        for (int d : devices) fn(d);
        return;
    }
    std::vector<std::thread> th;
    std::vector<std::exception_ptr> errs(devices.size());
    for (size_t i = 0; i < devices.size(); i++)
        th.emplace_back([&, i] {
            try {
                fn(devices[i]);
            } catch (...) {
                errs[i] = std::current_exception();
            }
        });
    for (auto& t : th) t.join();
    for (auto& e : errs)
        if (e) std::rethrow_exception(e);
}

struct msm_ticket_t;
template <class F>
struct bases_handle_t {
    std::vector<aff_mem_t<F>*> d;
    size_t n = 0;
    int tables = 1;
    int table_bits = 256;
    mutable std::mutex co_mu;
    mutable std::condition_variable co_cv;
    mutable std::deque<msm_ticket_t*> co_q;
    mutable int co_leaders = 0;
    void free_all() {
        int prev = 0;
        (void)hipGetDevice(&prev);
        for (size_t i = 0; i < d.size(); i++)
            if (d[i]) {
                (void)hipSetDevice(g_rt.devs[i]->physical);
                (void)hipFree(d[i]);
                d[i] = nullptr;
            }
        (void)hipSetDevice(prev);
    }
};
struct snarkvm_hip_bases : bases_handle_t<fq_t> {};

static const uint64_t FQ_R[6] = {202099033278250856ull,  5854854902718660529ull, 11492539364873682930ull,
                                 8885205928937022213ull, 5545221690922665192ull, 39800542322357402ull};
template <class F>
static void write_infinity(void* out) {
    const size_t fb = sizeof(typename F::mem_t);
    memset(out, 0, 3 * fb);
    memcpy((uint8_t*)out + fb, FQ_R, 48);
}

static constexpr int MSM_MAX_POS = 320;
template <class F>
struct msm_accum_t {
    xyzz_t<F> at[MSM_MAX_POS];
    bool used[MSM_MAX_POS];
    int top = -1;
    msm_accum_t() {
        for (int i = 0; i < MSM_MAX_POS; i++) used[i] = false;
    }
    void add(int pos, const xyzz_t<F>& p) {
        if (p.is_inf()) return;
        if (pos < 0 || pos >= MSM_MAX_POS) throw std::runtime_error("msm: bit position out of range");
        if (!used[pos]) {
            at[pos] = p;
            used[pos] = true;
        } else {
            at[pos].add(p);
        }
        if (pos > top) top = pos;
    }
    void finish(void* out) const {
        xyzz_t<F> t = xyzz_t<F>::inf();
        for (int p = top; p >= 0; p--) {
            t = t.dbl();
            if (used[p]) t.add(at[p]);
        }
        const jac_t<F> j = t.to_jacobian();
        uint32_t w[3 * F::MEM_WORDS];
        j.x.to_raw_words(w);
        j.y.to_raw_words(w + F::MEM_WORDS);
        j.z.to_raw_words(w + 2 * F::MEM_WORDS);
        memcpy(out, w, sizeof w);
    }
};
struct msm_pending_t {
    const void* planes = nullptr;
    int nplanes = 0;
    int tail_windows = 0, nbits = 0;
    int c = 0, m = 0;
    bool folded = false;
    int ninst = 0;
    bool lazy = false;
    int pos(int idx) const {
        const int tw = idx / nbits, j = idx % nbits;
        if (ninst) return (tw & 1) * m + j;
        return folded ? c * (tw >> 1) + (tw & 1) * m + j : c * tw + j;
    }
};
template <class F>
static constexpr size_t msm_point_bytes() {
    return sizeof(F) == sizeof(fq_t) && sizeof(xyzz_mem_t<fqz_t>) > sizeof(xyzz_mem_t<F>) ? sizeof(xyzz_mem_t<fqz_t>) : sizeof(xyzz_mem_t<F>);
}
template <class F>
static xyzz_t<F> msm_plane(const msm_pending_t& pd, int i) {
    if constexpr (sizeof(F) == sizeof(fq_t)) {
        if (pd.lazy) {
// ... 93 lines not shown
        const dim3 plane_grid((unsigned)g.nbits, (unsigned)g.tail_windows);
        hipLaunchKernelGGL((msm_bitplane_kernel<F, true>), plane_grid, dim3(plane_threads), 0, st, (const xyzz_mem_t<F>*)c.fold_sums.as<xyzz_mem_t<F>>(),
                           (const uint32_t*)nullptr, (const uint32_t*)nullptr, c.planes.as<xyzz_mem_t<F>>(), pl.nb, g.fold_m, g.fold_hb, hex, quads_planes, plane_flags);
        if constexpr (TAIL_FLAGGED<F>::value)
            hipLaunchKernelGGL((msm_bitplane_fix_kernel<F, true>), plane_grid, dim3(64), 0, st, (const xyzz_mem_t<F>*)c.fold_sums.as<xyzz_mem_t<F>>(), (const uint32_t*)nullptr,
                               (const uint32_t*)nullptr, c.planes.as<xyzz_mem_t<F>>(), pl.nb, g.fold_m, g.fold_hb, (const uint32_t*)plane_flags);
    } else {
        const dim3 plane_grid((unsigned)g.nbits, (unsigned)g.tail_windows);
        hipLaunchKernelGGL((msm_bitplane_kernel<F, false>), plane_grid, dim3(256), 0, st, sums, start, cnt, c.planes.as<xyzz_mem_t<F>>(), pl.nb, 0, 0, hex, 0, plane_flags);
        if constexpr (TAIL_FLAGGED<F>::value)
            hipLaunchKernelGGL((msm_bitplane_fix_kernel<F, false>), plane_grid, dim3(64), 0, st, sums, start, cnt, c.planes.as<xyzz_mem_t<F>>(), pl.nb, 0, 0,
                               (const uint32_t*)plane_flags);
    }
    HIP_TRY(hipGetLastError());
    HIP_TRY(hipMemcpyAsync(host_planes, c.planes.p, (size_t)pd.nplanes * sizeof(xyzz_mem_t<F>), hipMemcpyDeviceToHost, st));
}
struct msm_bucket_sink_t {
    void* acc = nullptr;
    uint32_t L = 1, slot = 0, nbt = 0;
    hipEvent_t after = nullptr, done = nullptr;
};
static int msm_trace_level() {
    static const int level = getenv("SNARKVM_HIP_TRACE") ? atoi(getenv("SNARKVM_HIP_TRACE")) : 0;
    return level;
}
struct msm_phases_t {
    lane_t& c;
    bool profile;
    int trace;
    size_t n;
    const char* cur = "";
    void begin(const char* name) {
        cur = name;
        if (trace >= 2) fprintf(stderr, "[snarkvm_hip] msm n=%zu: %s ...\n", n, name);
        if (profile) c.phase_begin(name);
    }
    void end() {
        if (profile) c.phase_end();
        if (trace >= 2) {
            const hipError_t e = hipStreamSynchronize(c.stream);
            fprintf(stderr, "[snarkvm_hip] msm n=%zu: %s done (%s)\n", n, cur, hipGetErrorString(e));
        }
    }
};
template <class T>
static void msm_reduce_and_tail(lane_t& c, const msm_plan_t& pl, const msm_tail_geom_t& tg, uint32_t nwin, uint32_t nbt, int rounds, size_t T0_max, size_t T1_max,
                                const msm_bucket_sink_t* sink, msm_pending_t& pd, void* host_planes, msm_phases_t& ph) {
    hipStream_t st = c.stream;
    ph.begin("msm_reduce_partials");
    uint32_t *cnt_in = c.cnt_a.as<uint32_t>(), *cnt_out = c.cnt_b.as<uint32_t>();
    uint32_t *start_in = c.start_a.as<uint32_t>(), *start_out = c.start_b.as<uint32_t>();
    xyzz_mem_t<T> *pin = c.part_a.as<xyzz_mem_t<T>>(), *pout = c.part_b.as<xyzz_mem_t<T>>();
    size_t T_in_max = T0_max;
    for (int r = 0; r < rounds; r++) {
        size_t T_out_max = T_in_max / pl.S2 + nbt + 1;
        if (T_out_max > T1_max) T_out_max = T1_max;
        hipLaunchKernelGGL(msm_alloc_kernel, dim3((nbt + 1 + 255) / 256), dim3(256), 0, st, cnt_in, cnt_out, nbt, pl.S2);
        exclusive_scan_u32(st, cnt_out, start_out, (size_t)nbt + 1, c.scan_tmp.as<uint32_t>());
        hipLaunchKernelGGL((msm_reduce_kernel<T>), dim3((unsigned)((T_out_max + 255) / 256)), dim3(256), 0, st, pin, start_in, cnt_in, start_out, pout, nbt,
                           pl.S2);
        std::swap(cnt_in, cnt_out);
        std::swap(start_in, start_out);
        std::swap(pin, pout);
        T_in_max = T_out_max;
    }
    ph.end();
    if (sink) {
        ph.begin("msm_bucket_merge");
        if (sink->after) HIP_TRY(hipStreamWaitEvent(st, sink->after, 0));
        hipLaunchKernelGGL((msm_bucket_merge_kernel<T>), dim3((nbt + 255) / 256), dim3(256), 0, st, (const xyzz_mem_t<T>*)pin, (const uint32_t*)start_in,
                           (const uint32_t*)cnt_in, (xyzz_mem_t<T>*)sink->acc, nbt, sink->L, sink->slot);
        if (sink->done) HIP_TRY(hipEventRecord(sink->done, st));
        ph.end();
        HIP_TRY(hipGetLastError());
        pd.nplanes = 0;
        return;
    }
    ph.begin("msm_bucket_reduce");
    msm_tail_launch<T>(c, pl, tg, nwin, nbt, pin, start_in, cnt_in, pd, host_planes);
    ph.end();
}
template <class F>
static void msm_launch_accumulate(lane_t& c, const msm_plan_t& pl, const aff_mem_t<F>* vbase, uint32_t* boffp, uint32_t nbt, size_t nthreads, bool one_wave,
                                  bool ltail) {
    hipStream_t st = c.stream;
#ifdef SV_BENCH
    static const uint32_t dbg_mask = getenv("SNARKVM_HIP_DEBUG_IDX_MASK") ? (uint32_t)strtoul(getenv("SNARKVM_HIP_DEBUG_IDX_MASK"), nullptr, 0) : 0xffffffffu;
#else
    constexpr uint32_t dbg_mask = 0xffffffffu;
#endif
    const size_t tmax = nthreads + nbt + 1;
    if constexpr (sizeof(F) == sizeof(fq_t)) {
        if (msm_lazy_on<F>()) {
            if (!ltail) c.part_raw.ensure(tmax * sizeof(g1_lazy_partial_t));
            g1_lazy_partial_t* raw_out = ltail ? c.part_a.as<g1_lazy_partial_t>() : c.part_raw.as<g1_lazy_partial_t>();
            hipLaunchKernelGGL((msm_accumulate_lazy_kernel<true>), dim3((unsigned)((nthreads + 255) / 256)), dim3(256), one_wave || tuning().acc_one_wg ? msm_acc_lds() : 0, st,
                               vbase, c.sorted.as<uint32_t>(), boffp, c.start_a.as<uint32_t>(), raw_out, nbt, pl.S, dbg_mask);
            if (!ltail)
                hipLaunchKernelGGL(g1_partials_to_exact_kernel, dim3((unsigned)((tmax + 255) / 256)), dim3(256), 0, st, (const g1_lazy_partial_t*)raw_out,
                                   c.part_a.as<g1_xyzz_mem_t>(), (const uint32_t*)c.start_a.as<uint32_t>(), nbt);
            return;
        }
    } else {
#ifndef SV_NO_G2
        if (msm_lazy_on<F>()) {
            c.part_raw.ensure(tmax * sizeof(g2_pair_partial_t));
            hipLaunchKernelGGL((msm_accumulate_pair2_kernel<false>), dim3((unsigned)((2 * nthreads + 255) / 256)), dim3(256), 0, st, vbase, c.sorted.as<uint32_t>(),
                               boffp, c.start_a.as<uint32_t>(), c.part_raw.as<g2_pair_partial_t>(), nbt, pl.S, dbg_mask);
            hipLaunchKernelGGL(g2_pair_partials_to_exact_kernel, dim3((unsigned)((8 * tmax + 255) / 256)), dim3(256), 0, st,
                               (const g2_pair_partial_t*)c.part_raw.as<g2_pair_partial_t>(), c.part_a.as<xyzz_mem_t<fq2_t>>(),
                               (const uint32_t*)c.start_a.as<uint32_t>(), nbt);
            return;
        }
#endif
    }
    if (one_wave)
        hipLaunchKernelGGL((msm_accumulate_seg_kernel<F, 1, true>), dim3((unsigned)((nthreads + 255) / 256)), dim3(256), 0, st, vbase, c.sorted.as<uint32_t>(), boffp,
                           c.start_a.as<uint32_t>(), c.part_a.as<xyzz_mem_t<F>>(), nbt, pl.S, dbg_mask);
    else
        hipLaunchKernelGGL((msm_accumulate_seg_kernel<F, 1, false>), dim3((unsigned)((nthreads + 255) / 256)), dim3(256), 0, st, vbase, c.sorted.as<uint32_t>(), boffp,
                           c.start_a.as<uint32_t>(), c.part_a.as<xyzz_mem_t<F>>(), nbt, pl.S, dbg_mask);
}
template <class F>
static size_t msm_plane_bytes() {
    return (size_t)MSM_MAX_POS * msm_point_bytes<F>();
}
template <class F>
struct msm_job_t {
    const aff_mem_t<F>* bases = nullptr;
    const aff_mem_t<F>* bases1 = nullptr;
    size_t n0 = 0;
    int tables = 1;
    size_t table_stride = 0;
    int table_bits = 0;
    const uint4* scalars = nullptr;
    size_t n = 0;
    int scalars_montgomery = 0;
    int window_bits = 0;
    void* host_planes = nullptr;
    bool profile = true;
    const msm_multi_t* multi = nullptr;
    const msm_bucket_sink_t* sink = nullptr;
    hipEvent_t scalars_read = nullptr;
};
template <class F>
struct msm_layout_t {
    msm_plan_t pl;
    bool wide;
    bool fused;
    bool ltail;
    bool single_round, prefetch_ok;
    uint32_t nwin, nbt;
    size_t E_max, T0_max, T1_max;
    const aff_mem_t<F>* vbase;
    msm_tail_geom_t tg;
    msm_radix_params_t rp;
    msm_digit_params_t dp;
    int LBL;
    uint32_t B1, nbins, nseg_last;
    size_t ncounts1, tiles1, tiles2_max;
};
template <class F>
static msm_layout_t<F> msm_layout(lane_t& c, const msm_job_t<F>& j, msm_pending_t& pd) {
    const msm_multi_t* mu = j.multi;
    const size_t n = j.n;
    size_t n0 = j.bases1 ? j.n0 : n;
    if (n0 > n) n0 = n;
    msm_layout_t<F> L{};
    if (n >= ((size_t)1 << 31)) throw hip_failure{hipErrorInvalidValue, "msm: npoints must be < 2^31", __LINE__};
    const msm_plan_t pl = L.pl = msm_make_plan(n, mu ? j.table_bits : j.window_bits, j.tables, j.table_bits);
    L.wide = pl.c > 16;
    if (mu && (L.wide || pl.W != 1 || pl.c < 12 || (size_t)pl.J * mu->hn >= ((size_t)1 << 31) || n != mu->npad || n % SORT_TILE))
        throw hip_failure{hipErrorInvalidValue, "msm: geometry not eligible for a fused multi-instance run", __LINE__};
    if ((size_t)pl.Wd * n >= ((size_t)1 << 32)) throw hip_failure{hipErrorInvalidValue, "msm: windows * npoints must be < 2^32", __LINE__};
    if ((size_t)pl.J * n >= ((size_t)1 << 31)) throw hip_failure{hipErrorInvalidValue, "msm: tables * npoints must be < 2^31", __LINE__};
    const aff_mem_t<F>* vb1 = j.bases1 ? j.bases1 : j.bases;
    L.vbase = mu ? j.bases : (vb1 < j.bases ? vb1 : j.bases);
    if (!mu) {
        const size_t top0 = (size_t)(j.bases - L.vbase) + n0, top1 = (size_t)(vb1 - L.vbase) + (n - n0);
        if ((size_t)(pl.J - 1) * j.table_stride + (top0 > top1 ? top0 : top1) >= ((size_t)1 << 31))
            throw hip_failure{hipErrorInvalidValue, "msm: base slots must be addressable in 31 bits (tables * registered points < 2^31)", __LINE__};
    }
    const size_t E_max = L.E_max = (size_t)pl.Wd * n;
    const uint32_t nwin = L.nwin = mu ? mu->K : (uint32_t)pl.W;
    const uint32_t nbt = L.nbt = nwin * pl.nb;

    c.scan_tmp.ensure((scan_tmp_elems((size_t)nbt + 1)) * 4);
    c.boff.ensure(((size_t)nbt + 2) * 4);
    c.cnt_a.ensure(((size_t)nbt + 1) * 4);
    c.cnt_b.ensure(((size_t)nbt + 1) * 4);
    c.start_a.ensure(((size_t)nbt + 1) * 4);
    c.start_b.ensure(((size_t)nbt + 1) * 4);
    const size_t slack = (size_t)nbt / 32 + 64;
    L.T0_max = E_max / pl.S + nbt + 1 + slack;
    L.T1_max = L.T0_max / pl.S2 + nbt + 1 + slack;
    pd.lazy = L.ltail = msm_lazy_tail_on<F>();
    c.part_a.ensure(L.T0_max * msm_partial_bytes<F>());
    c.part_b.ensure(L.T1_max * msm_partial_bytes<F>());
    L.tg = msm_tail_geometry(pl, nwin, pd, mu ? (int)mu->K : 0);
    if (mu && (size_t)pd.nplanes > mu->plane_capacity) throw hip_failure{hipErrorInvalidValue, "msm: plane staging of the fused group too small", __LINE__};
    if (j.sink && (mu || j.sink->nbt != nbt)) throw hip_failure{hipErrorInvalidValue, "msm: bucket sink does not match the plan", __LINE__};
    c.planes.ensure((size_t)pd.nplanes * msm_partial_bytes<F>());

    L.fused = !mu && L.wide && tuning().fused && pl.c <= 22 && pl.Wd <= FUSED_MAX_ROWS;
    memcpy(L.dp.bias, pl.bias, sizeof L.dp.bias);
    L.dp.c = pl.c;
    L.dp.W = pl.Wd;
    L.dp.n = n;
    L.dp.montgomery = j.scalars_montgomery;
    L.single_round = mu || (size_t)pl.Wd * n <= ((size_t)1 << 22);
    L.prefetch_ok = (size_t)pl.Wd * n <= ((size_t)1 << 22);

    msm_radix_params_t& rp = L.rp;
    rp.n = n;
    rp.c = pl.c;
    rp.W = pl.W;
    rp.J = pl.J;
// ... 120 lines not shown
    if (j.multi)
        hipLaunchKernelGGL(radix_bin_layout_multi_kernel, dim3((L.nbins + 1 + 255) / 256), dim3(256), 0, st, off1, counts1, L.ncounts1,
                           c.rbinstart.as<uint32_t>(), L.nbins, L.rp);
    else
        hipLaunchKernelGGL(radix_bin_layout_kernel, dim3((L.nbins + 1 + 255) / 256), dim3(256), 0, st, off1, counts1, L.ncounts1, c.rbinstart.as<uint32_t>(),
                           L.nbins, L.rp.TPW);
    ph.end();
}
static void msm_tile_segments(lane_t& c, const uint32_t* seg_start, uint32_t nseg) {
    hipLaunchKernelGGL(radix_bin_tiles_kernel, dim3((nseg + 1 + 255) / 256), dim3(256), 0, c.stream, seg_start, c.rntiles.as<uint32_t>(), nseg);
    exclusive_scan_u32(c.stream, c.rntiles.as<uint32_t>(), c.rtstart.as<uint32_t>(), (size_t)nseg + 1, c.scan_tmp.as<uint32_t>());
}
static void msm_colscan(lane_t& c, uint32_t* sizes, uint32_t nsegs, int bits, uint32_t* dmax) {
    if (nsegs <= 4096)
        hipLaunchKernelGGL(radix_colscan2_seg_kernel, dim3(nsegs), dim3(1024), 0, c.stream, c.rcounts2.as<uint32_t>(), c.roff2.as<uint32_t>(),
                           c.rtstart.as<uint32_t>(), sizes, nsegs, bits, dmax);
    else
        hipLaunchKernelGGL(radix_colscan2_kernel, dim3(((nsegs << bits) + 1 + 255) / 256), dim3(256), 0, c.stream, c.rcounts2.as<uint32_t>(),
                           c.roff2.as<uint32_t>(), c.rtstart.as<uint32_t>(), sizes, nsegs, bits, dmax);
}
template <class F>
static void msm_stage_sort_rest(lane_t& c, const msm_layout_t<F>& L, msm_phases_t& ph) {
    hipStream_t st = c.stream;
    const size_t E_max = L.E_max;
    const uint32_t nbt = L.nbt;
    uint32_t* bsize = c.rbsize.as<uint32_t>();
    uint32_t* d_max = bsize + nbt + 1;
    uint32_t* boffp = c.boff.as<uint32_t>();
    const uint32_t* seg_start = c.rbinstart.as<uint32_t>();
    uint32_t nseg = L.nbins;
    const uint32_t* v_in = c.rv1.as<uint32_t>();
    if (L.wide) {
        ph.begin("msm_sort_level2");
        const uint32_t ngroups = nseg << 7;
        const size_t tmax = E_max / SORT_TILE + nseg + 1;
        c.rv2.ensure(E_max * 4);
        c.rl2.ensure(E_max);
        c.rmid_size.ensure(((size_t)ngroups + 3) * 4);
        c.rmid_boff.ensure(((size_t)ngroups + 3) * 4);
        c.scan_tmp.ensure(scan_tmp_elems((size_t)ngroups + 2) * 4);
        uint32_t* msize = c.rmid_size.as<uint32_t>();
        uint32_t* mboff = c.rmid_boff.as<uint32_t>();
        msm_tile_segments(c, seg_start, nseg);
        hipLaunchKernelGGL((radix_hist2_kernel<uint16_t>), dim3((unsigned)tmax), dim3(SORT_THREADS), 0, st, c.rl1.as<uint16_t>(), seg_start,
                           c.rtstart.as<uint32_t>(), c.rcounts2.as<uint32_t>(), nseg, 7, 7);
        HIP_TRY(hipMemsetAsync(msize + ngroups + 1, 0, 4, st));
        msm_colscan(c, msize, nseg, 7, msize + ngroups + 1);
        exclusive_scan_u32(st, msize, mboff, (size_t)ngroups + 1, c.scan_tmp.as<uint32_t>());
        hipLaunchKernelGGL((radix_scatter2_kernel<uint16_t, uint8_t>), dim3((unsigned)tmax), dim3(SORT_THREADS), 0, st, v_in, c.rl1.as<uint16_t>(),
                           seg_start, c.rtstart.as<uint32_t>(), c.rcounts2.as<uint32_t>(), c.roff2.as<uint32_t>(), mboff, c.rv2.as<uint32_t>(),
                           c.rl2.as<uint8_t>(), nseg, 7, 7, (uint32_t)tuning().xcd);
        ph.end();
        seg_start = mboff;
        nseg = ngroups;
        v_in = c.rv2.as<uint32_t>();
    }
    ph.begin(L.wide ? "msm_sort_level3" : "msm_sort_level2");
    msm_tile_segments(c, seg_start, nseg);
    const uint8_t* rem_last = L.wide ? c.rl2.as<uint8_t>() : c.rl1.as<uint8_t>();
    hipLaunchKernelGGL((radix_hist2_kernel<uint8_t>), dim3((unsigned)L.tiles2_max), dim3(SORT_THREADS), 0, st, rem_last, seg_start,
                       c.rtstart.as<uint32_t>(), c.rcounts2.as<uint32_t>(), nseg, L.LBL, 0);
    HIP_TRY(hipMemsetAsync(d_max, 0, 4, st));
    msm_colscan(c, bsize, nseg, L.LBL, d_max);
    exclusive_scan_u32(st, bsize, boffp, (size_t)nbt + 1, c.scan_tmp.as<uint32_t>());
    hipLaunchKernelGGL((radix_scatter2_kernel<uint8_t, uint8_t>), dim3((unsigned)L.tiles2_max), dim3(SORT_THREADS), 0, st, v_in, rem_last, seg_start,
                       c.rtstart.as<uint32_t>(), c.rcounts2.as<uint32_t>(), c.roff2.as<uint32_t>(), boffp, c.sorted.as<uint32_t>(),
                       (uint8_t*)nullptr, nseg, L.LBL, 0, (uint32_t)tuning().xcd);
    ph.end();
}
template <class F>
static int msm_stage_accumulate(lane_t& c, const msm_layout_t<F>& L, const msm_job_t<F>& j, msm_phases_t& ph) {
    hipStream_t st = c.stream;
    const msm_multi_t* mu = j.multi;
    const uint32_t nbt = L.nbt;
    uint32_t* boffp = c.boff.as<uint32_t>();
    int rounds = 0;
    ph.begin("msm_accumulate");
    const int env_rounds = tuning().reduce_rounds;
    if (!L.single_round) rounds = env_rounds < 0 ? 0 : (env_rounds > 8 ? 8 : env_rounds);
    if (mu && tuning().fuse_reduce > 0) rounds = tuning().fuse_reduce > 4 ? 4 : tuning().fuse_reduce;
    if (mu && tuning().fuse_reduce < 0) rounds = mu->K >= 8 ? 1 : 0;
    hipLaunchKernelGGL(msm_alloc_seg_kernel, dim3((nbt + 1 + 255) / 256), dim3(256), 0, st, boffp, c.cnt_a.as<uint32_t>(), nbt, L.pl.S);
    exclusive_scan_u32(st, c.cnt_a.as<uint32_t>(), c.start_a.as<uint32_t>(), (size_t)nbt + 1, c.scan_tmp.as<uint32_t>());
    msm_launch_accumulate<F>(c, L.pl, L.vbase, boffp, nbt, (L.E_max + L.pl.S - 1) / L.pl.S, L.single_round && L.prefetch_ok, L.ltail);
    ph.end();
    return rounds;
}
template <class T>
struct msm_field_tag {
    using type = T;
};
template <class F, class Fn>
static void msm_on_tail_field(bool lazy, Fn&& fn) {
    if constexpr (sizeof(F) == sizeof(fq_t)) {
        if (lazy) return fn(msm_field_tag<fqz_t>{});
    }
    fn(msm_field_tag<F>{});
}
template <class F>
static msm_pending_t msm_run(lane_t& c, const msm_job_t<F>& j) {
    msm_pending_t pd;
    pd.planes = j.host_planes;
    if (j.n == 0) return pd;
    msm_phases_t ph{c, j.profile, msm_trace_level(), j.n};
    const msm_layout_t<F> L = msm_layout(c, j, pd);
    if (!L.fused) msm_stage_digits(c, L, j, ph);
    msm_stage_level1(c, L, j, ph);
    msm_stage_sort_rest(c, L, ph);
    const int rounds = msm_stage_accumulate(c, L, j, ph);
    msm_on_tail_field<F>(L.ltail, [&](auto t) {
        msm_reduce_and_tail<typename decltype(t)::type>(c, L.pl, L.tg, L.nwin, L.nbt, rounds, L.T0_max, L.T1_max, j.sink, pd, j.host_planes, ph);
    });
    return pd;
}
template <class F>
static msm_pending_t msm_tail_from_sink(lane_t& c, const msm_job_t<F>& j, const msm_bucket_sink_t& sink) {
    msm_pending_t pd;
    pd.planes = j.host_planes;
    const msm_plan_t pl = msm_make_plan(j.n, j.window_bits, j.tables, j.table_bits);
    const uint32_t nwin = (uint32_t)pl.W, nbt = nwin * pl.nb;
    if (nbt != sink.nbt) throw hip_failure{hipErrorInvalidValue, "msm: bucket sink does not match the plan", __LINE__};
    const msm_tail_geom_t tg = msm_tail_geometry(pl, nwin, pd, 0);
    c.start_a.ensure(((size_t)nbt + 1) * 4);
    c.cnt_a.ensure(((size_t)nbt + 1) * 4);
    hipLaunchKernelGGL(msm_sink_lists_kernel, dim3((nbt + 1 + 255) / 256), dim3(256), 0, c.stream, c.start_a.as<uint32_t>(), c.cnt_a.as<uint32_t>(), nbt, sink.L);
    pd.lazy = msm_lazy_tail_on<F>();
    c.phase_begin("msm_bucket_reduce");
    msm_on_tail_field<F>(pd.lazy, [&](auto t) {
        using T = typename decltype(t)::type;
        msm_tail_launch<T>(c, pl, tg, nwin, nbt, (const xyzz_mem_t<T>*)sink.acc, c.start_a.as<uint32_t>(), c.cnt_a.as<uint32_t>(), pd, j.host_planes);
    });
    c.phase_end();
    return pd;
}
template <class F>
static void msm_run_sync(lane_t& c, const msm_job_t<F>& j, void* out) {
    if (c.in_scope && c.pin_used) scope_flush();
    c.pin.ensure(msm_plane_bytes<F>());
    msm_job_t<F> staged = j;
    staged.host_planes = c.pin.p;
    const msm_pending_t pd = msm_run<F>(c, staged);
    HIP_TRY(hipStreamSynchronize(c.stream));
    const double t0 = host_now_ms();
    msm_accum_t<F>* acc = new msm_accum_t<F>();
    std::unique_ptr<msm_accum_t<F>> hold(acc);
    msm_collect<F>(*acc, pd);
    acc->finish(out);
    c.phase_host("msm_host_finish", host_now_ms() - t0);
}

template <class F>
static bool msm_lazy_on() {
    return sizeof(F) == sizeof(fq_t) ? tuning().lazy != 0 : tuning().lazy2 != 0;
}
template <class F>
static void convert_bases(lane_t& c, const uint8_t* d_in, size_t stride, size_t n, aff_mem_t<F>* d_out, hipStream_t st = nullptr, bool for_msm = false) {
    if (!n) return;
    const int form406 = for_msm && msm_lazy_on<F>() ? 1 : 0;
    hipLaunchKernelGGL((convert_bases_kernel<F>), dim3((unsigned)((n + 255) / 256)), dim3(256), 0, st ? st : c.stream, d_in, stride, n, d_out, form406);
    HIP_TRY(hipGetLastError());
}
static void bases_to_lazy_form(lane_t& c, g1_aff_mem_t* d, size_t slots) {
    if (!slots || !msm_lazy_on<fq_t>()) return;
    hipLaunchKernelGGL(g1_bases_to_form406_kernel, dim3((unsigned)((slots + 255) / 256)), dim3(256), 0, c.stream, d, slots);
    HIP_TRY(hipGetLastError());
}
#ifndef SV_NO_G2
static void bases_to_lazy_form(lane_t& c, aff_mem_t<fq2_t>* d, size_t slots) {
    if (!slots || !msm_lazy_on<fq2_t>()) return;
    hipLaunchKernelGGL(g2_bases_to_form406_kernel, dim3((unsigned)((slots + 255) / 256)), dim3(256), 0, c.stream, d, slots);
    HIP_TRY(hipGetLastError());
}
#endif

template <class F>
static void precompute_tables_run(lane_t& c, aff_mem_t<F>* d, size_t n, int tables, int table_bits) {
    if (tables <= 1 || !n) return;
    int run = (int)(n >> 16);
    run = run < 1 ? 1 : (run > PRE_RUN ? PRE_RUN : run);
    const size_t slab = n < PRE_SLAB ? n : PRE_SLAB;
    c.gen_pts.ensure(4 * slab * sizeof(typename F::mem_t));
    for (int j = 1; j < tables; j++)
        for (size_t lo = 0; lo < n; lo += PRE_SLAB) {
            const size_t cnt = n - lo < PRE_SLAB ? n - lo : PRE_SLAB;
            const size_t threads = (cnt + run - 1) / run;
            hipLaunchKernelGGL((precompute_table_kernel<F>), dim3((unsigned)((threads + 255) / 256)), dim3(256), 0, c.stream, d + (size_t)(j - 1) * n + lo,
                               d + (size_t)j * n + lo, cnt, table_bits, run, (typename F::mem_t*)c.gen_pts.p);
        }
    HIP_TRY(hipGetLastError());
}

static int batch_lanes(size_t npoints) {
    const int env = tuning().lanes;
    int l = env > 0 ? env : (npoints >= ((size_t)1 << 20) ? 3 : 8);
    return l < 1 ? 1 : (l > device_t::LANES ? device_t::LANES : l);
}
static constexpr size_t MSM_SPLIT_MIN = (size_t)1 << 18;
static size_t msm_chunk_pairs() {
    const int lg = tuning().msm_chunk_lg;
    return (size_t)1 << (lg < 16 ? 16 : (lg > 30 ? 30 : lg));
}
static size_t msm_scalar_chunk_pairs() {
    const int lg = tuning().scalar_chunk_lg;
    return (size_t)1 << (lg < 18 ? 18 : lg > 30 ? 30 : lg);
}

template <class Upload, class Compute>
static void lane_ring_run(lane_guard& lg, size_t count, Upload&& upload, Compute&& compute, int trace, double t_begin) {
    const size_t L = lg.lanes.size();
    const int phys = lg.lanes[0]->dev->physical;
    std::mutex mu;
    std::condition_variable cv;
    std::vector<char> uploaded(count, 0), enqueued(count, 0);
    std::vector<hipEvent_t> up(count), used(count);
    for (size_t j = 0; j < count; j++) {
        up[j] = lg.lanes[j % L]->new_event();
        used[j] = lg.lanes[j % L]->new_event();
    }
    std::exception_ptr up_err, cp_err;
    std::thread uploader([&] {
        try {
            HIP_TRY(hipSetDevice(phys));
            for (size_t j = 0; j < count; j++) {
                lane_t& c = *lg.lanes[j % L];
                if (j >= L) {
                    char state;
                    {
                        std::unique_lock<std::mutex> lk(mu);
                        cv.wait(lk, [&] { return enqueued[j - L] != 0; });
                        state = enqueued[j - L];
                    }
                    if (state == 2) break;
                    HIP_TRY(hipEventSynchronize(used[j - L]));
                }
                const double t0 = host_now_ms();
                upload(j, c.alt);
                HIP_TRY(hipEventRecord(up[j], c.alt));
                if (trace) fprintf(stderr, "[snarkvm_hip] chunk %zu dev %d lane %d: uploaded t+%.2f .. t+%.2f ms\n", j, c.dev->logical, c.index, t0 - t_begin, host_now_ms() - t_begin);
                {
                    std::lock_guard<std::mutex> lk(mu);
                    uploaded[j] = 1;
                }
                cv.notify_all();
            }
        } catch (...) {
            up_err = std::current_exception();
            std::lock_guard<std::mutex> lk(mu);
            for (auto& u : uploaded) u = 2;
            cv.notify_all();
        }
    });
    try {
        for (size_t j = 0; j < count; j++) {
            lane_t& c = *lg.lanes[j % L];
            {
                std::unique_lock<std::mutex> lk(mu);
                cv.wait(lk, [&] { return uploaded[j] != 0; });
                if (uploaded[j] == 2) break;
            }
            HIP_TRY(hipStreamWaitEvent(c.stream, up[j], 0));
            const double t0 = host_now_ms();
            compute(j);
            HIP_TRY(hipEventRecord(used[j], c.stream));
            if (trace) fprintf(stderr, "[snarkvm_hip] chunk %zu: enqueued t+%.2f .. t+%.2f ms\n", j, t0 - t_begin, host_now_ms() - t_begin);
            {
                std::lock_guard<std::mutex> lk(mu);
                enqueued[j] = 1;
            }
            cv.notify_all();
        }
    } catch (...) {
// ... 101 lines not shown
            uint8_t* raw = c.bases_tmp.template as<uint8_t>() + aff_bytes;
            HIP_TRY(hipMemcpyAsync(raw, (const uint8_t*)points + chunk_lo(j) * stride, chunk_cnt(j) * stride, hipMemcpyHostToDevice, st));
            HIP_TRY(hipMemcpyAsync(c.scalars_tmp.p, (const uint8_t*)scalars + chunk_lo(j) * 32, chunk_cnt(j) * 32, hipMemcpyHostToDevice, st));
        };
        auto compute = [&](size_t j, bool prof) {
            lane_t& c = *lg.lanes[j % L];
            uint8_t* raw = c.bases_tmp.template as<uint8_t>() + aff_bytes;
            if (prof) c.phase_begin("msm_convert_bases");
            convert_bases<F>(c, raw, stride, chunk_cnt(j), c.bases_tmp.template as<aff_mem_t<F>>(), nullptr, true);
            if (prof) c.phase_end();
            msm_bucket_sink_t mine_sink = sink;
            mine_sink.slot = (uint32_t)(j % L);
            msm_job_t<F> job;
            job.bases = c.bases_tmp.template as<aff_mem_t<F>>();
            job.scalars = c.scalars_tmp.template as<uint4>();
            job.n = chunk_cnt(j);
            job.window_bits = chunk_c;
            job.host_planes = c.pin.template as<uint8_t>() + (use_sink ? 0 : slot * (j / L));
            job.profile = prof;
            job.sink = use_sink ? &mine_sink : nullptr;
            const msm_pending_t pd = msm_run<F>(c, job);
            if (!use_sink) pend[j] = pd;
        };
        if (mine.size() == 1) {
            lane_t& c = *lg.lanes[0];
            c.phase_begin("msm_h2d");
            upload(0, c.stream);
            c.phase_end();
            compute(0, true);
        } else {
            lane_ring_run(lg, mine.size(), upload, [&](size_t j) { compute(j, false); }, trace, t_begin);
        }
        if (use_sink) {
            lane_t& c0 = *lg.lanes[0];
            for (int l = 1; l < L; l++) {
                hipEvent_t e = lg.lanes[l]->new_event();
                HIP_TRY(hipEventRecord(e, lg.lanes[l]->stream));
                HIP_TRY(hipStreamWaitEvent(c0.stream, e, 0));
            }
            msm_job_t<F> tail;
            tail.n = max_cnt;
            tail.window_bits = chunk_c;
            tail.host_planes = c0.pin.p;
            pend[0] = msm_tail_from_sink<F>(c0, tail, sink);
        }
        for (int l = 0; l < L; l++) {
            HIP_TRY(hipStreamSynchronize(lg.lanes[l]->alt));
            HIP_TRY(hipStreamSynchronize(lg.lanes[l]->stream));
        }
        const double t_sync = host_now_ms();
        {
            std::lock_guard<std::mutex> lk(acc_mu);
            for (auto& pd : pend) msm_collect<F>(*acc, pd);
        }
        if (trace) fprintf(stderr, "[snarkvm_hip] all chunks done at t+%.2f ms, planes collected in %.2f ms\n", t_sync - t_begin, host_now_ms() - t_sync);
        for (int l = 0; l < L; l++) lg.lanes[l]->end_call();
    });
    acc->finish(out);
}

static constexpr size_t MSM_FUSE_MAX_PAIRS = (size_t)1 << 18;
static constexpr size_t MSM_FUSE_MAX_ENTRIES = (size_t)1 << 26;
static bool msm_fuse_enabled() {
    return tuning().fuse_batch != 0;
}
static size_t msm_fuse_max_k() {
    const int k = tuning().fuse_max_k;
    return (size_t)(k < 2 ? 2 : (k > 256 ? 256 : k));
}
struct msm_req_t {
    size_t off0 = 0, n0 = 0, off1 = 0, n1 = 0;
    const void* scalars = nullptr;
    void* out = nullptr;
};
template <class F>
static msm_job_t<F> msm_handle_job(const bases_handle_t<F>& h, int dev, const msm_req_t& r) {
    msm_job_t<F> j;
    j.bases = h.d[dev] + r.off0;
    j.bases1 = r.n1 ? h.d[dev] + r.off1 : nullptr;
    j.n0 = r.n0;
    j.tables = h.tables;
    j.table_stride = h.n;
    j.table_bits = h.table_bits;
    j.n = r.n0 + r.n1;
    return j;
}
template <class Fn>
static void host_parallel_for(size_t n, int max_threads, Fn fn) {
    size_t T = n / 4;
    if (T > (size_t)max_threads) T = (size_t)max_threads;
    if (T <= 1) {
        for (size_t i = 0; i < n; i++) fn(i);
        return;
    }
    std::atomic<size_t> next{0};
    std::vector<std::exception_ptr> errs(T);
    auto work = [&](size_t t) {
        try {
            for (size_t i; (i = next.fetch_add(1)) < n;) fn(i);
        } catch (...) {
            errs[t] = std::current_exception();
        }
    };
    std::vector<std::thread> th;
    for (size_t t = 1; t < T; t++) th.emplace_back(work, t);
    work(0);
    for (auto& x : th) x.join();
    for (auto& e : errs)
        if (e) std::rethrow_exception(e);
}
template <class F>
static bool msm_handle_fusable(const bases_handle_t<F>& h, int window_bits) {
    if (!msm_fuse_enabled() || h.tables <= 1 || h.table_bits < 12 || h.table_bits > 16 || (window_bits != 0 && window_bits != h.table_bits) ||
        (size_t)h.tables * h.n >= ((size_t)1 << 31) || h.n >= ((size_t)1 << 31))
        return false;
    const msm_plan_t pl = msm_make_plan(SORT_TILE, h.table_bits, h.tables, h.table_bits);
    return pl.W == 1 && pl.c == h.table_bits;
}
template <class F>
static size_t msm_fuse_planes(const bases_handle_t<F>& h) {
    return 2 * ((size_t)h.table_bits / 2 + 1);
}
static size_t msm_padded(size_t n) { return (n + SORT_TILE - 1) / SORT_TILE * SORT_TILE; }
template <class F>
static std::vector<std::vector<size_t>> msm_make_jobs(const bases_handle_t<F>& h, const msm_req_t* req, const std::vector<size_t>& mine, bool fusable_handle) {
    std::vector<std::vector<size_t>> jobs;
    std::vector<size_t> group;
    size_t group_entries = 0;
    auto flush = [&] {
        if (!group.empty()) jobs.push_back(group);
        group.clear();
        group_entries = 0;
    };
    for (size_t k : mine) {
        const size_t tot = req[k].n0 + req[k].n1;
        const bool small = fusable_handle && tot > 0 && tot <= MSM_FUSE_MAX_PAIRS;
        if (!small) {
            jobs.push_back({k});
            continue;
        }
        const size_t e = msm_padded(tot) * (size_t)h.tables;
        if (!group.empty() && (group.size() >= msm_fuse_max_k() || group_entries + e > MSM_FUSE_MAX_ENTRIES)) flush();
        group.push_back(k);
        group_entries += e;
    }
    flush();
    return jobs;
}
template <class F>
static void msm_job_staging(const bases_handle_t<F>& h, const std::vector<size_t>& job, size_t& plane_bytes, size_t& table_bytes) {
    const size_t K = job.size();
    plane_bytes = K > 1 ? K * msm_fuse_planes(h) * msm_point_bytes<F>() : msm_plane_bytes<F>();
    table_bytes = K > 1 ? ((K + 1) * sizeof(msm_inst_t) + 255) / 256 * 256 : 0;
}
template <class F>
static msm_pending_t msm_enqueue_job(lane_t& c, const bases_handle_t<F>& h, int dev, const msm_req_t* req, const std::vector<size_t>& job, uint8_t* host_planes,
                                     msm_inst_t* tab, int scalars_on_device, int scalars_montgomery, int window_bits, hipEvent_t scalars_read = nullptr) {
    if (job.size() == 1) {
        const msm_req_t& r = req[job[0]];
        const size_t n = r.n0 + r.n1;
        const uint4* d_sc = (const uint4*)r.scalars;
        if (!scalars_on_device && n) {
            c.scalars.ensure(n * 32);
            HIP_TRY(hipMemcpyAsync(c.scalars.p, r.scalars, n * 32, hipMemcpyHostToDevice, c.stream));
            d_sc = c.scalars.template as<uint4>();
        }
// ... 436 lines not shown
```

snarkvm_amd/csrc/tuning.hip.h:

```cpp
#pragma once
#include <stdio.h>
#include <stdlib.h>
#include <string.h>

namespace sv {

struct tuning_t {
    int lazy = 1, lazy2 = 1, fused = 1;
    long acc_lds = 96 * 1024;
    int acc_one_wg = 0, reduce_rounds = 1, fuse_batch = 1, fuse_max_k = 64, fuse_reduce = -1, coalesce = 1, coalesce_us = 40, lanes = 0;
    int msm_chunk_lg = 20, scalar_chunk_lg = 22, taper = 1, ring_lanes = 3, seg = 0, seg2 = 0, fold_l = 0, scan1 = 1;
    int ntt_min_tiles = 256, ntt_full_tw = 1, ntt_fold = 1, ntt_batch = 1;
    int xcd = 1, fold_threads2 = 128, coalesce_slots = 2, ramp = 3, scalar_geo = 4, lazy_tail = 1, horner2 = 1, hex2 = 1, group_quad = 1, tail_quads = 13, fold_small2 = 256, fold_mid = 128;

    bool set(const char* key, long v) {
#define SV_TUNE_KEY(name)                  \
    if (!strcmp(key, #name)) {             \
        name = (decltype(name))v;          \
        return true;                       \
    }
        SV_TUNE_KEY(lazy) SV_TUNE_KEY(lazy2) SV_TUNE_KEY(fused) SV_TUNE_KEY(acc_lds)
        SV_TUNE_KEY(acc_one_wg) SV_TUNE_KEY(reduce_rounds) SV_TUNE_KEY(fuse_batch) SV_TUNE_KEY(fuse_max_k) SV_TUNE_KEY(fuse_reduce) SV_TUNE_KEY(coalesce)
        SV_TUNE_KEY(coalesce_us) SV_TUNE_KEY(lanes) SV_TUNE_KEY(msm_chunk_lg) SV_TUNE_KEY(scalar_chunk_lg) SV_TUNE_KEY(taper) SV_TUNE_KEY(ring_lanes) SV_TUNE_KEY(seg) SV_TUNE_KEY(seg2)
        SV_TUNE_KEY(fold_l) SV_TUNE_KEY(scan1) SV_TUNE_KEY(ntt_min_tiles) SV_TUNE_KEY(ntt_full_tw) SV_TUNE_KEY(ntt_fold)
        SV_TUNE_KEY(ntt_batch) SV_TUNE_KEY(xcd) SV_TUNE_KEY(fold_threads2) SV_TUNE_KEY(coalesce_slots) SV_TUNE_KEY(ramp) SV_TUNE_KEY(scalar_geo) SV_TUNE_KEY(lazy_tail) SV_TUNE_KEY(horner2) SV_TUNE_KEY(hex2) SV_TUNE_KEY(group_quad) SV_TUNE_KEY(tail_quads) SV_TUNE_KEY(fold_small2) SV_TUNE_KEY(fold_mid)
#undef SV_TUNE_KEY
        return false;
    }
    void parse(const char* s) {
        while (s && *s) {
            while (*s == ',' || *s == ' ') s++;
            const char* eq = strchr(s, '=');
            const char* end = strchr(s, ',');
            if (!end) end = s + strlen(s);
            if (!*s) break;
            char key[32] = {0};
            if (!eq || eq > end || (size_t)(eq - s) >= sizeof key) {
                fprintf(stderr, "[snarkvm_hip] SNARKVM_HIP_TUNING: malformed item at \"%s\" (ignored)\n", s);
            } else {
                memcpy(key, s, (size_t)(eq - s));
                char* num_end = nullptr;
                const long v = strtol(eq + 1, &num_end, 0);
                if (num_end == eq + 1 || !set(key, v)) fprintf(stderr, "[snarkvm_hip] SNARKVM_HIP_TUNING: unknown key or bad value \"%s\" (ignored)\n", key);
            }
            s = end;
        }
    }
    void clamp() {
        auto fix = [](const char* key, auto& v, long lo, long hi) {
            if ((long)v < lo || (long)v > hi) {
                const long was = (long)v;
                v = (decltype(v + 0))((long)v < lo ? lo : hi);
                fprintf(stderr, "[snarkvm_hip] SNARKVM_HIP_TUNING: %s=%ld is out of range [%ld, %ld]; using %ld\n", key, was, lo, hi, (long)v);
            }
        };
        fix("coalesce_slots", coalesce_slots, 1, 8);
        fix("coalesce_us", coalesce_us, 0, 100000);
        fix("fuse_max_k", fuse_max_k, 2, 256);
        fix("fuse_reduce", fuse_reduce, -1, 4);
        fix("reduce_rounds", reduce_rounds, 0, 8);
        fix("lanes", lanes, 0, 8);
        fix("ring_lanes", ring_lanes, 2, 8);
        fix("ntt_min_tiles", ntt_min_tiles, 1, 1 << 20);
        fix("acc_lds", acc_lds, 0, 160 * 1024);
        fix("msm_chunk_lg", msm_chunk_lg, 16, 30);
        fix("scalar_chunk_lg", scalar_chunk_lg, 18, 30);
        fix("ramp", ramp, 0, 6);
        fix("scalar_geo", scalar_geo, 0, 16);
        fix("seg", seg, 0, 4096);
        fix("seg2", seg2, 0, 256);
        fix("fold_l", fold_l, 0, 64);
    }
};
inline const tuning_t& tuning() {
    static const tuning_t t = [] {
        tuning_t v;
        v.parse(getenv("SNARKVM_HIP_TUNING"));
        v.clamp();
        return v;
    }();
    return t;
}

}
```

snarkvm_amd/msm.py:

```python
import ctypes

import numpy as np

from . import _lib, plugin
from .layout import G1_AFFINE, G1_PROJECTIVE


class VariableBase:
    @staticmethod
    def msm(bases, scalars):
        return plugin.msm(bases, scalars)


class RegisteredBases:

    def __init__(self, bases=None, device_ptr=None, npoints=None, tables=1, window_bits=0):
        L = _lib.lib()
        self._h = ctypes.c_void_p()
        self.tables = int(tables)
        self.window_bits = int(window_bits)
        if device_ptr is not None:
            self.n = int(npoints)
            src, on_device = ctypes.c_void_p(device_ptr), 1
        else:
            bases = np.ascontiguousarray(bases, dtype=G1_AFFINE).reshape(-1)
            self.n = bases.shape[0]
            src, on_device = ctypes.c_void_p(bases.ctypes.data), 0
        if self.window_bits:
            err = L.snarkvm_hip_register_bases_windowed(ctypes.byref(self._h), src, ctypes.c_size_t(self.n), ctypes.c_size_t(G1_AFFINE.itemsize),
                                                        ctypes.c_int(on_device), ctypes.c_int(self.tables), ctypes.c_int(self.window_bits))
        else:
            err = L.snarkvm_hip_register_bases_tables(ctypes.byref(self._h), src, ctypes.c_size_t(self.n), ctypes.c_size_t(G1_AFFINE.itemsize),
                                                      ctypes.c_int(on_device), ctypes.c_int(self.tables))
        _lib.check(err)

    @classmethod
    def from_serialized(cls, data, npoints, compressed=False, validate=False, tables=1):
        from . import serialize

        self = cls.__new__(cls)
        self.tables = int(tables)
        self.window_bits = 0
        self.n = int(npoints)
        self._h = serialize.register_bases_serialized(data, npoints, compressed, validate, tables)
        return self

    def msm(self, scalars=None, offset=0, device_ptr=None, npoints=None, window_bits=0):
        L = _lib.lib()
        out = np.zeros(1, dtype=G1_PROJECTIVE)
        if device_ptr is not None:
            n = int(npoints)
            err = L.snarkvm_hip_msm_registered(ctypes.c_void_p(out.ctypes.data), self._h, ctypes.c_size_t(offset), ctypes.c_size_t(n),
                                               ctypes.c_void_p(device_ptr), ctypes.c_int(1), ctypes.c_int(window_bits))
        else:
            scalars = np.ascontiguousarray(scalars, dtype=np.uint64).reshape(-1, 4)
            n = scalars.shape[0]
            err = L.snarkvm_hip_msm_registered(ctypes.c_void_p(out.ctypes.data), self._h, ctypes.c_size_t(offset), ctypes.c_size_t(n),
                                               ctypes.c_void_p(scalars.ctypes.data), ctypes.c_int(0), ctypes.c_int(window_bits))
        _lib.check(err)
        return out

    def msm_batch(self, scalars_list=None, offsets=None, device_ptrs=None, npoints=None, window_bits=0, montgomery=False):
        L = _lib.lib()
        if device_ptrs is not None:
            count = len(device_ptrs)
            ns = [int(v) for v in npoints]
            ptrs = [int(p) for p in device_ptrs]
            on_dev = 1
            keep = None
        else:
            keep = [np.ascontiguousarray(s, dtype=np.uint64).reshape(-1, 4) for s in scalars_list]
            count = len(keep)
            ns = [k.shape[0] for k in keep]
            ptrs = [k.ctypes.data for k in keep]
            on_dev = 0
        offs = [0] * count if offsets is None else [int(o) for o in offsets]
        out = np.zeros(count, dtype=G1_PROJECTIVE)
        c_offs = (ctypes.c_size_t * max(1, count))(*offs)
        c_ns = (ctypes.c_size_t * max(1, count))(*ns)
        c_ptrs = (ctypes.c_void_p * max(1, count))(*ptrs)
        _lib.check(L.snarkvm_hip_msm_registered_batch(ctypes.c_void_p(out.ctypes.data), self._h, ctypes.c_size_t(count), c_offs, c_ns, c_ptrs,
                                                      ctypes.c_int(on_dev), ctypes.c_int(1 if montgomery else 0), ctypes.c_int(window_bits)))
        return out

    def close(self):
        if self._h:
            _lib.lib().snarkvm_hip_free_bases(self._h)
            self._h = ctypes.c_void_p()

    def __del__(self):
        try:
            self.close()
        except Exception:
            pass


def msm_g2(bases, scalars):
    from .layout import G2_AFFINE, G2_PROJECTIVE

    bases = np.ascontiguousarray(bases, dtype=G2_AFFINE).reshape(-1)
    scalars = np.ascontiguousarray(scalars, dtype=np.uint64).reshape(-1, 4)
    n = scalars.shape[0]
    if n > bases.shape[0]:
        raise ValueError(f"length mismatch {bases.shape[0]} points < {n} scalars")
    out = np.zeros(1, dtype=G2_PROJECTIVE)
    err = _lib.lib().snarkvm_hip_msm_g2(ctypes.c_void_p(out.ctypes.data), ctypes.c_void_p(bases.ctypes.data), ctypes.c_size_t(n),
                                        ctypes.c_void_p(scalars.ctypes.data), ctypes.c_size_t(G2_AFFINE.itemsize))
    _lib.check(err)
    return out


class RegisteredBasesG2:

    def __init__(self, bases, tables=16, window_bits=0):
        from .layout import G2_AFFINE

        bases = np.ascontiguousarray(bases, dtype=G2_AFFINE).reshape(-1)
        self.n = bases.shape[0]
        self._h = ctypes.c_void_p()
        _lib.check(_lib.lib().snarkvm_hip_register_bases_g2(ctypes.byref(self._h), ctypes.c_void_p(bases.ctypes.data), ctypes.c_size_t(self.n),
                                                           ctypes.c_size_t(G2_AFFINE.itemsize), ctypes.c_int(int(tables)), ctypes.c_int(int(window_bits))))

    def msm(self, scalars=None, offset=0, window_bits=0, device_ptr=None, npoints=None):
        from .layout import G2_PROJECTIVE

        out = np.zeros(1, dtype=G2_PROJECTIVE)
        if device_ptr is not None:
            _lib.check(_lib.lib().snarkvm_hip_msm_g2_registered(ctypes.c_void_p(out.ctypes.data), self._h, ctypes.c_size_t(offset),
# ... 57 lines not shown
```

Before: 550.7 million pairs/s.

## Store registered G1 base tables in twisted Edwards form for bucket accumulation

At registration, each precomputed G1 base table is converted from short-Weierstrass affine into extended twisted Edwards slots (y-x, y+x, 2dxy), using a batched inversion per thread run. It first runs a subgroup-membership check unless membership was already proven, and keeps the old affine layout as a fallback. The MSM accumulate step then uses a new Edwards bucket kernel and converts the partial sums back to XYZZ. The goal is cheaper unified mixed additions in the bucket phase. The cost is slower registration with a membership check, larger 192-byte slots that add memory traffic, and a new code path that can affect correctness.

```diff
diff --git a/include/snarkvm_hip.h b/include/snarkvm_hip.h
--- a/include/snarkvm_hip.h
+++ b/include/snarkvm_hip.h
@@ -68,6 +68,7 @@
 RustError snarkvm_hip_register_bases_windowed(snarkvm_hip_bases_t **handle, const void *points, size_t npoints,
                                               size_t ffi_affine_sz, int on_device, int tables, int window_bits);
 void snarkvm_hip_free_bases(snarkvm_hip_bases_t *handle);
+int snarkvm_hip_bases_form(const snarkvm_hip_bases_t *handle);
 
 RustError snarkvm_hip_register_bases_serialized(snarkvm_hip_bases_t **handle, const void *bytes, size_t npoints,
                                                 int compressed, int validate, int tables);
diff --git a/rust/snarkvm-algorithms-hip/src/sys.rs b/rust/snarkvm-algorithms-hip/src/sys.rs
--- a/rust/snarkvm-algorithms-hip/src/sys.rs
+++ b/rust/snarkvm-algorithms-hip/src/sys.rs
@@ -52,6 +52,7 @@
     pub fn snarkvm_hip_register_bases_tables(handle: *mut *mut snarkvm_hip_bases_t, points: *const c_void, npoints: usize, ffi_affine_sz: usize, on_device: i32, tables: i32) -> Error;
     pub fn snarkvm_hip_register_bases_windowed(handle: *mut *mut snarkvm_hip_bases_t, points: *const c_void, npoints: usize, ffi_affine_sz: usize, on_device: i32, tables: i32, window_bits: i32) -> Error;
     pub fn snarkvm_hip_free_bases(handle: *mut snarkvm_hip_bases_t);
+    pub fn snarkvm_hip_bases_form(handle: *const snarkvm_hip_bases_t) -> i32;
     pub fn snarkvm_hip_register_bases_serialized(handle: *mut *mut snarkvm_hip_bases_t, bytes: *const c_void, npoints: usize, compressed: i32, validate: i32, tables: i32) -> Error;
     pub fn snarkvm_hip_g1_deserialize(out_affine: *mut c_void, bytes: *const c_void, n: usize, compressed: i32, validate: i32) -> Error;
     pub fn snarkvm_hip_g1_serialize(out_bytes: *mut c_void, affine: *const c_void, n: usize, ffi_affine_sz: usize, compressed: i32) -> Error;
diff --git a/snarkvm_amd/_lib.py b/snarkvm_amd/_lib.py
--- a/snarkvm_amd/_lib.py
+++ b/snarkvm_amd/_lib.py
@@ -9,7 +9,7 @@
     "snarkvm_hip_device_count", "snarkvm_hip_batch_lanes", "snarkvm_hip_set_device", "snarkvm_hip_set_devices", "snarkvm_hip_num_devices",
     "snarkvm_hip_malloc", "snarkvm_hip_free", "snarkvm_hip_memcpy_h2d", "snarkvm_hip_memcpy_d2h", "snarkvm_hip_memcpy_d2d", "snarkvm_hip_memset", "snarkvm_hip_ntt_device", "snarkvm_hip_ntt_device_batch", "snarkvm_hip_polymul_device",
     "snarkvm_hip_scope_begin", "snarkvm_hip_scope_end", "snarkvm_hip_scope_begin_ex", "snarkvm_hip_scope_collect", "snarkvm_hip_scope_set_flags", "snarkvm_hip_scope_stream", "snarkvm_hip_alloc_stats",
-    "snarkvm_hip_register_bases", "snarkvm_hip_register_bases_tables", "snarkvm_hip_register_bases_windowed", "snarkvm_hip_free_bases", "snarkvm_hip_msm_registered", "snarkvm_hip_msm_g2",
+    "snarkvm_hip_register_bases", "snarkvm_hip_register_bases_tables", "snarkvm_hip_register_bases_windowed", "snarkvm_hip_free_bases", "snarkvm_hip_bases_form", "snarkvm_hip_msm_registered", "snarkvm_hip_msm_g2",
     "snarkvm_hip_msm_registered_ex", "snarkvm_hip_msm_registered_batch", "snarkvm_hip_msm_registered_batch_ex", "snarkvm_hip_g1_to_affine",
     "snarkvm_hip_fr_mul_device", "snarkvm_hip_fr_convert_device", "snarkvm_hip_g1_generate_bases_device",
     "snarkvm_hip_fr_vec_op", "snarkvm_hip_fr_divide_by_linear", "snarkvm_hip_fr_batch_inversion_and_mul",
@@ -91,6 +91,8 @@
         L.snarkvm_hip_selftest_g1_msm_naive.restype = ctypes.c_int
         L.snarkvm_hip_selftest_msm_plan.restype = ctypes.c_int
         L.snarkvm_hip_free_bases.restype = None
+        L.snarkvm_hip_bases_form.restype = ctypes.c_int
+        L.snarkvm_hip_bases_form.argtypes = [ctypes.c_void_p]
         L.snarkvm_hip_free_bases_g2.restype = None
         L.snarkvm_hip_set_profiling.restype = None
         L.snarkvm_hip_coalescer_stats.restype = None
diff --git a/snarkvm_amd/csrc/api.hip b/snarkvm_amd/csrc/api.hip
--- a/snarkvm_amd/csrc/api.hip
+++ b/snarkvm_amd/csrc/api.hip
@@ -3,6 +3,7 @@
 #include "ffl.hip.h"
 
 runtime_t g_rt;
+int sv_g1_finish_registration(lane_t& c, snarkvm_hip_bases* h, int dev, g1_aff_mem_t* table0, bool members_proved, bool edwards_ok);
 thread_local thread_scope_t g_tl_scope;
 thread_scope_t::~thread_scope_t() {
     if (!lane) return;
@@ -261,7 +262,7 @@
 
 static void precompute_tables(lane_t& c, snarkvm_hip_bases* h, g1_aff_mem_t* d) { precompute_tables_run<fq_t>(c, d, h->n, h->tables, h->table_bits); }
 static void register_bases_impl(snarkvm_hip_bases_t** handle, const void* points, size_t npoints, size_t ffi_affine_sz, int on_device, int tables,
-                                int table_bits) {
+                                int table_bits, bool edwards_ok = true) {
     if (!handle) throw hip_failure{hipErrorInvalidValue, "register_bases: null handle", __LINE__};
     if (npoints && !points) throw hip_failure{hipErrorInvalidValue, "register_bases: null points", __LINE__};
     if (ffi_affine_sz < 104 || (ffi_affine_sz & 7)) throw hip_failure{hipErrorInvalidValue, "register_bases: bad stride", __LINE__};
@@ -273,31 +274,38 @@
     h->tables = tables;
     h->table_bits = table_bits ? table_bits : 256 / tables;
     h->d.assign(nd, nullptr);
-    const size_t bytes = (size_t)tables * npoints * sizeof(g1_aff_mem_t);
+    std::vector<int> forms(nd, 0);
     try {
         if (npoints) {
             const int owner = on_device ? device_for(points, 1) : -1;
             auto build = [&](int dev) {
                 lane_guard lg(dev);
                 lane_t& c = lg.c();
-                HIP_TRY(hipMalloc((void**)&h->d[dev], bytes));
+                g1_aff_mem_t* table0 = nullptr;
+                HIP_TRY(hipMalloc((void**)&table0, npoints * sizeof(g1_aff_mem_t)));
                 const uint8_t* src = (const uint8_t*)points;
-                if (!on_device) {
-                    c.bases_tmp.ensure(npoints * ffi_affine_sz);
-                    HIP_TRY(hipMemcpyAsync(c.bases_tmp.p, points, npoints * ffi_affine_sz, hipMemcpyHostToDevice, c.stream));
-                    src = c.bases_tmp.as<uint8_t>();
+                try {
+                    if (!on_device) {
+                        c.bases_tmp.ensure(npoints * ffi_affine_sz);
+                        HIP_TRY(hipMemcpyAsync(c.bases_tmp.p, points, npoints * ffi_affine_sz, hipMemcpyHostToDevice, c.stream));
+                        src = c.bases_tmp.as<uint8_t>();
+                    }
+                    convert_bases<fq_t>(c, src, ffi_affine_sz, npoints, table0);
+                } catch (...) {
+                    (void)hipFree(table0);
+                    throw;
                 }
-                convert_bases<fq_t>(c, src, ffi_affine_sz, npoints, h->d[dev]);
-                precompute_tables(c, h.get(), h->d[dev]);
-                bases_to_lazy_form(c, h->d[dev], (size_t)tables * npoints);
-                HIP_TRY(hipStreamSynchronize(c.stream));
+                forms[dev] = sv_g1_finish_registration(c, h.get(), dev, table0, false, edwards_ok);
             };
             std::vector<int> all;
             for (int d = 0; d < nd; d++) all.push_back(d);
             if (!on_device) {
                 for_each_device(all, build);
+                h->form = forms[0];
             } else {
                 build(owner);
+                h->form = forms[owner];
+                const size_t bytes = (size_t)tables * npoints * (h->form ? sizeof(g1_ed_slot_t) : sizeof(g1_aff_mem_t));
                 for (int d = 0; d < nd; d++) {
                     if (d == owner) continue;
                     lane_guard lg(d);
@@ -346,6 +354,7 @@
     return h;
 }
 void sv_precompute_tables(lane_t& c, snarkvm_hip_bases* h, g1_aff_mem_t* d) { precompute_tables(c, h, d); }
+extern "C" int snarkvm_hip_bases_form(const snarkvm_hip_bases_t* handle) { return handle ? handle->form : 0; }
 extern "C" {
 
 static void check_window_bits(int window_bits, const char* who) {
@@ -783,7 +792,7 @@
                     verify_pool().submit(job);
                     job->wait();
                 }
-                register_bases_impl(&nh, points, npoints, stride, 0, tables, bits);
+                register_bases_impl(&nh, points, npoints, stride, 0, tables, bits, false);
             } catch (...) {
                 (void)hipGetLastError();
                 g_base_cache[i].failed = true;
diff --git a/snarkvm_amd/csrc/api_serde.hip b/snarkvm_amd/csrc/api_serde.hip
--- a/snarkvm_amd/csrc/api_serde.hip
+++ b/snarkvm_amd/csrc/api_serde.hip
@@ -2,6 +2,108 @@
 
 snarkvm_hip_bases* sv_new_bases_handle(size_t npoints, int tables, int table_bits);
 void sv_precompute_tables(lane_t& c, snarkvm_hip_bases* h, g1_aff_mem_t* d);
+
+static __global__ void __launch_bounds__(64) g1_bases_membership_kernel(const g1_aff_mem_t* __restrict__ bases, size_t n, uint32_t* __restrict__ failed) {
+    const size_t i = blockIdx.x * (size_t)blockDim.x + threadIdx.x;
+    if (i >= n) return;
+    const g1_aff_t p = g1_load_aff(&bases[i]);
+    if (p.is_inf()) return;
+    if (!g1_is_on_curve(p) || !g1_is_in_subgroup(p)) atomicOr(failed, 1u);
+}
+static __global__ void __launch_bounds__(256) g1_table_to_edwards_kernel(const g1_aff_mem_t* __restrict__ table, g1_ed_slot_t* __restrict__ out, size_t n, int run,
+                                                                  fq_t::mem_t* __restrict__ scratch) {
+    const size_t t = blockIdx.x * (size_t)blockDim.x + threadIdx.x;
+    const size_t first = t * (size_t)run;
+    if (first >= n) return;
+    const size_t cnt = n - first < (size_t)run ? n - first : (size_t)run;
+    const fq_t s = fq_t::from_table(FqEd::S377), one = fq_t::one();
+    auto uvw = [&](const g1_aff_t& p, fq_t& u, fq_t& v) -> fq_t {
+        u = s * (p.x + one);
+        v = s * p.y;
+        return p.is_inf() ? fq_t::zero() : v * (u + one);
+    };
+    fq_t prod = one;
+    for (size_t i = 0; i < cnt; i++) {
+        fq_t u, v;
+        const fq_t w = uvw(g1_load_aff(&table[first + i]), u, v);
+        if (!w.is_zero()) prod = prod * w;
+        prod.store(&scratch[first + i]);
+    }
+    fq_t inv = prod.inverse();
+    const fq_t f = fq_t::from_table(FqEd::F377), two_d = fq_t::from_table(FqEd::TWO_D377), c406 = fq_t::from_table(FqLConv::C406);
+    for (size_t i = cnt; i-- > 0;) {
+        fq_t u, v;
+        const fq_t w = uvw(g1_load_aff(&table[first + i]), u, v);
+        if (w.is_zero()) {
+            g1_ed_slot_t::store_identity(&out[first + i]);
+            continue;
+        }
+        const fq_t before = i == 0 ? one : fq_t::load(&scratch[first + i - 1]);
+        const fq_t wi = inv * before;
+        inv = inv * w;
+        const fq_t xe = f * u * (wi * (u + one));
+        const fq_t ye = (u - one) * (wi * v);
+        g1_ed_slot_t::store(&out[first + i], (ye - xe) * c406, (ye + xe) * c406, (two_d * xe * ye) * c406);
+    }
+}
+struct dev_owned_t {
+    void* p = nullptr;
+    ~dev_owned_t() {
+        if (p) (void)hipFree(p);
+    }
+    void* release() {
+        void* q = p;
+        p = nullptr;
+        return q;
+    }
+};
+int sv_g1_finish_registration(lane_t& c, snarkvm_hip_bases* h, int dev, g1_aff_mem_t* table0, bool members_proved, bool edwards_ok) {
+    dev_owned_t t0, t1, slots;
+    t0.p = table0;
+    const size_t n = h->n;
+    const int tables = h->tables;
+    int form = edwards_ok && tuning().edwards != 0 && msm_lazy_on<fq_t>() ? 1 : 0;
+    if (form && !members_proved) {
+        c.serde_status.ensure(4);
+        HIP_TRY(hipMemsetAsync(c.serde_status.p, 0, 4, c.stream));
+        hipLaunchKernelGGL(g1_bases_membership_kernel, dim3((unsigned)((n + 63) / 64)), dim3(64), 0, c.stream, (const g1_aff_mem_t*)table0, n, c.serde_status.as<uint32_t>());
+        HIP_TRY(hipGetLastError());
+        uint32_t failed = 0;
+        HIP_TRY(hipMemcpyAsync(&failed, c.serde_status.p, 4, hipMemcpyDeviceToHost, c.stream));
+        HIP_TRY(hipStreamSynchronize(c.stream));
+        if (failed) form = 0;
+    }
+    if (form) {
+        HIP_TRY(hipMalloc(&slots.p, (size_t)tables * n * sizeof(g1_ed_slot_t)));
+        if (tables > 1) HIP_TRY(hipMalloc(&t1.p, n * sizeof(g1_aff_mem_t)));
+        const int run = precompute_run_length(n);
+        c.gen_prod.ensure((n < PRE_SLAB ? n : PRE_SLAB) * sizeof(fq_t::mem_t));
+        g1_aff_mem_t *cur = (g1_aff_mem_t*)t0.p, *other = (g1_aff_mem_t*)t1.p;
+        for (int j = 0; j < tables; j++) {
+            for (size_t lo = 0; lo < n; lo += PRE_SLAB) {
+                const size_t cnt = n - lo < PRE_SLAB ? n - lo : PRE_SLAB;
+                const size_t threads = (cnt + run - 1) / run;
+                hipLaunchKernelGGL(g1_table_to_edwards_kernel, dim3((unsigned)((threads + 255) / 256)), dim3(256), 0, c.stream, (const g1_aff_mem_t*)cur + lo,
+                                   (g1_ed_slot_t*)slots.p + (size_t)j * n + lo, cnt, run, (fq_t::mem_t*)c.gen_prod.p);
+            }
+            if (j + 1 < tables) {
+                precompute_table_step<fq_t>(c, cur, other, n, h->table_bits);
+                std::swap(cur, other);
+            }
+        }
+        HIP_TRY(hipGetLastError());
+        HIP_TRY(hipStreamSynchronize(c.stream));
+        h->d[dev] = (g1_aff_mem_t*)slots.release();
+        return 1;
+    }
+    HIP_TRY(hipMalloc(&slots.p, (size_t)tables * n * sizeof(g1_aff_mem_t)));
+    HIP_TRY(hipMemcpyAsync(slots.p, table0, n * sizeof(g1_aff_mem_t), hipMemcpyDeviceToDevice, c.stream));
+    sv_precompute_tables(c, h, (g1_aff_mem_t*)slots.p);
+    bases_to_lazy_form(c, (g1_aff_mem_t*)slots.p, (size_t)tables * n);
+    HIP_TRY(hipStreamSynchronize(c.stream));
+    h->d[dev] = (g1_aff_mem_t*)slots.release();
+    return 0;
+}
 
 static uint32_t g1_deserialize_run(lane_t& c, const void* bytes, size_t n, int compressed, int validate, g1_aff_mem_t* d_native, uint8_t* d_rust) {
     const size_t psz = compressed ? 48 : 96;
@@ -30,15 +132,16 @@
         try {
             std::vector<int> all;
             for (int d = 0; d < g_rt.ndev(); d++) all.push_back(d);
+            std::vector<int> forms(g_rt.ndev(), 0);
             for_each_device(all, [&](int dev) {
                 lane_guard lg(dev);
                 lane_t& c = lg.c();
-                HIP_TRY(hipMalloc((void**)&h->d[dev], (size_t)tables * npoints * sizeof(g1_aff_mem_t)));
-                serde_throw_on_status(g1_deserialize_run(c, bytes, npoints, compressed, validate, h->d[dev], nullptr), "register_bases_serialized");
-                sv_precompute_tables(c, h.get(), h->d[dev]);
-                bases_to_lazy_form(c, h->d[dev], (size_t)tables * npoints);
-                HIP_TRY(hipStreamSynchronize(c.stream));
+                dev_owned_t t0;
+                HIP_TRY(hipMalloc(&t0.p, npoints * sizeof(g1_aff_mem_t)));
+                serde_throw_on_status(g1_deserialize_run(c, bytes, npoints, compressed, validate, (g1_aff_mem_t*)t0.p, nullptr), "register_bases_serialized");
+                forms[dev] = sv_g1_finish_registration(c, h.get(), dev, (g1_aff_mem_t*)t0.release(), validate != 0, true);
             });
+            h->form = forms[0];
         } catch (...) {
             h->free_all();
             throw;
diff --git a/snarkvm_amd/csrc/ffl.hip.h b/snarkvm_amd/csrc/ffl.hip.h
--- a/snarkvm_amd/csrc/ffl.hip.h
+++ b/snarkvm_amd/csrc/ffl.hip.h
@@ -359,6 +359,131 @@
     }
 };
 
+struct FqEd {
+    static constexpr int32_t S406[13] = {0x08449ac2, 0x16bc6341, 0x1f27346e, 0x003fa706, 0x16341794, 0x0e03035e, 0x1f0a2ed9, 0x0c4c0908, 0x1a0645ff, 0x0dd41749, 0x078fb647, 0x1b5db1c4, 0x1660c39d};
+    static constexpr int32_t F406[13] = {0x18d0ec00, 0x19d5ac0b, 0x099a00af, 0x14f3163d, 0x15201f1a, 0x185e2df4, 0x10000b58, 0x16cc24d5, 0x0cfaac7e, 0x1feb43c4, 0x0f6e64c6, 0x1143d6d9, 0x182ac132};
+    static constexpr uint32_t S377[13] = {0x15b06342u, 0x147204a9u, 0x175a8e5fu, 0x1b70ccaeu, 0x191d2c43u, 0x14f44be2u, 0x0c8e35beu, 0x04244b5fu, 0x03c7e17fu, 0x19c83ffeu, 0x04c75929u, 0x1ebe20cdu, 0x13f11581u};
+    static constexpr uint32_t F377[13] = {0x11d5ac0cu, 0x188710abu, 0x113a9644u, 0x0de71d1cu, 0x09f8a717u, 0x03256d6du, 0x0a20f9a6u, 0x135c575bu, 0x0d358eb7u, 0x0ade3d8du, 0x08f489cfu, 0x194e6931u, 0x06095b1du};
+    static constexpr uint32_t TWO_D377[13] = {0x08894e0eu, 0x11646fe8u, 0x107d548cu, 0x0dcd13a1u, 0x01bbf564u, 0x11bbc2a5u, 0x094c9893u, 0x1aa2ff5eu, 0x014482f8u, 0x175aa204u, 0x1dbaab07u, 0x117a94deu, 0x0c5e2f3cu};
+};
+
+struct alignas(64) g1_ed_slot_t {
+    uint32_t w[48];
+    SV_HD static void store(g1_ed_slot_t* slot, const fq_t& ym, const fq_t& yp, const fq_t& k) {
+        uint32_t t[48];
+#pragma unroll
+        for (int i = 0; i < 13; i++) t[i] = ym.v[i], t[13 + i] = yp.v[i], t[26 + i] = k.v[i];
+#pragma unroll
+        for (int i = 39; i < 48; i++) t[i] = 0;
+        uint4* q = (uint4*)slot;
+#pragma unroll
+        for (int i = 0; i < 12; i++) q[i] = make_uint4(t[4 * i], t[4 * i + 1], t[4 * i + 2], t[4 * i + 3]);
+    }
+    SV_HD static void store_identity(g1_ed_slot_t* slot) {
+        const fq_t one = fq_t::from_table(FqLConv::C406);
+        store(slot, one, one, fq_t::zero());
+    }
+};
+struct g1_ed_operand_t {
+    uint4 q[10];
+    SV_HD static g1_ed_operand_t load(const g1_ed_slot_t* slot) {
+        g1_ed_operand_t r;
+        const uint4* p = (const uint4*)slot;
+#pragma unroll
+        for (int i = 0; i < 10; i++) r.q[i] = p[i];
+        return r;
+    }
+    SV_HD void limbs(fql_t& ym, fql_t& yp, fql_t& k) const {
+        uint32_t t[40];
+#pragma unroll
+        for (int i = 0; i < 10; i++) t[4 * i] = q[i].x, t[4 * i + 1] = q[i].y, t[4 * i + 2] = q[i].z, t[4 * i + 3] = q[i].w;
+#pragma unroll
+        for (int i = 0; i < 13; i++) ym.v[i] = (int32_t)t[i], yp.v[i] = (int32_t)t[13 + i], k.v[i] = (int32_t)t[26 + i];
+        SV_OPAQUE_13(ym.v);
+        SV_OPAQUE_13(yp.v);
+        SV_OPAQUE_13(k.v);
+    }
+};
+
+struct ed_lazy_t {
+    fql_t x, y, z, t;
+
+    SV_HD static ed_lazy_t identity() {
+        ed_lazy_t r;
+        r.x = r.t = fql_t::zero();
+        r.y = r.z = xyzz_lazy_t::one();
+        return r;
+    }
+    SV_HD void madd(const fql_t& ym, const fql_t& yp, const fql_t& k, bool negate) {
+        fql_t m, p;
+#pragma unroll
+        for (int i = 0; i < fql_t::N; i++) m.v[i] = negate ? yp.v[i] : ym.v[i], p.v[i] = negate ? ym.v[i] : yp.v[i];
+        const fql_t a = fql_t::mul(y - x, m);
+        const fql_t b = fql_t::mul((y + x).normalized(), p);
+        const fql_t c = fql_t::mul(t, k.negate_if(negate));
+        fql_t f, g, h;
+        {
+            int32_t cf = 0, cg = 0, ch = 0;
+#pragma unroll
+            for (int i = 0; i < fql_t::N - 1; i++) {
+                const int32_t d = 2 * z.v[i];
+                const int32_t tf = d - c.v[i] + cf, tg = d + c.v[i] + cg, th = b.v[i] + a.v[i] + ch;
+                f.v[i] = (int32_t)((uint32_t)tf & fql_t::MASK), cf = tf >> 29;
+                g.v[i] = (int32_t)((uint32_t)tg & fql_t::MASK), cg = tg >> 29;
+                h.v[i] = (int32_t)((uint32_t)th & fql_t::MASK), ch = th >> 29;
+            }
+            constexpr int T = fql_t::N - 1;
+            f.v[T] = 2 * z.v[T] - c.v[T] + cf;
+            g.v[T] = 2 * z.v[T] + c.v[T] + cg;
+            h.v[T] = b.v[T] + a.v[T] + ch;
+            SV_OPAQUE_13(f.v);
+            SV_OPAQUE_13(g.v);
+            SV_OPAQUE_13(h.v);
+        }
+        const fql_t e = b - a;
+        x = fql_t::mul(e, f);
+        y = fql_t::mul(g, h);
+        t = fql_t::mul(e, h);
+        z = fql_t::mul(f, g);
+    }
+    SV_HD void store_raw(g1_lazy_partial_t* p) const {
+        uint4* q = (uint4*)p;
+        int32_t w[52];
+#pragma unroll
+        for (int i = 0; i < 13; i++) w[i] = x.v[i], w[13 + i] = y.v[i], w[26 + i] = z.v[i], w[39 + i] = t.v[i];
+#pragma unroll
+        for (int i = 0; i < 13; i++) q[i] = make_uint4((uint32_t)w[4 * i], (uint32_t)w[4 * i + 1], (uint32_t)w[4 * i + 2], (uint32_t)w[4 * i + 3]);
+    }
+    SV_HD void to_xyzz(fql_t& ox, fql_t& oy, fql_t& ozz, fql_t& ozzz) const {
+        fql_t cs, cf;
+#pragma unroll
+        for (int i = 0; i < fql_t::N; i++) cs.v[i] = FqEd::S406[i], cf.v[i] = FqEd::F406[i];
+        const fql_t sum = (z + y).normalized();
+        const fql_t sd = fql_t::mul(z - y, cs);
+        const fql_t zr = fql_t::mul(sd, x);
+        ozz = fql_t::sqr(zr);
+        ozzz = fql_t::mul(ozz, zr);
+        ox = fql_t::mul(fql_t::mul(sum - sd, x), zr);
+        oy = fql_t::mul(fql_t::mul(fql_t::mul(sum, z), cf), ozz);
+    }
+    SV_HD static void raw_to_xyzz(g1_lazy_partial_t* p) {
+        uint4* q = (uint4*)p;
+        int32_t w[52];
+#pragma unroll
+        for (int i = 0; i < 13; i++) {
+            const uint4 u = q[i];
+            w[4 * i] = (int32_t)u.x, w[4 * i + 1] = (int32_t)u.y, w[4 * i + 2] = (int32_t)u.z, w[4 * i + 3] = (int32_t)u.w;
+        }
+        ed_lazy_t e;
+#pragma unroll
+        for (int i = 0; i < 13; i++) e.x.v[i] = w[i], e.y.v[i] = w[13 + i], e.z.v[i] = w[26 + i], e.t.v[i] = w[39 + i];
+        xyzz_lazy_t r;
+        e.to_xyzz(r.x, r.y, r.zz, r.zzz);
+        r.inf = (((uint32_t)r.zz.v[0] + 8u) & fql_t::MASK) <= 16u && r.zz.to_exact().is_zero();
+        r.store_raw(p);
+    }
+};
+
 struct fqz_t {
     fql_t a;
     struct mem_t {
diff --git a/snarkvm_amd/csrc/msm_sort.hip.h b/snarkvm_amd/csrc/msm_sort.hip.h
--- a/snarkvm_amd/csrc/msm_sort.hip.h
+++ b/snarkvm_amd/csrc/msm_sort.hip.h
@@ -799,6 +799,72 @@
     }
 }
 
+#ifndef SV_ED_AHEAD
+#define SV_ED_AHEAD 1
+#endif
+#ifndef SV_ED_MINW
+#define SV_ED_MINW 1
+#endif
+template <bool PREFETCH>
+__global__ void __launch_bounds__(256, SV_ED_MINW) msm_accumulate_ed_kernel(const g1_ed_slot_t* __restrict__ bases, const uint32_t* __restrict__ sorted,
+                                                            const uint32_t* __restrict__ boff, const uint32_t* __restrict__ start,
+                                                            g1_lazy_partial_t* __restrict__ partial, uint32_t nbt, uint32_t S, uint32_t debug_idx_mask) {
+    const uint32_t t = blockIdx.x * blockDim.x + threadIdx.x;
+    const uint32_t total = boff[nbt];
+    const uint64_t lo64 = (uint64_t)t * S;
+    if (lo64 >= total) return;
+    const uint32_t lo = (uint32_t)lo64;
+    const uint32_t hi = (total - lo < S) ? total : lo + S;
+    uint32_t k = find_bucket(boff, nbt, lo);
+    uint32_t kend = boff[k + 1];
+    uint32_t kend2 = boff[k + 2 <= nbt ? k + 2 : nbt];
+    uint32_t start_k = start[k];
+    uint32_t part_off = t - boff[k] / S;
+    ed_lazy_t acc = ed_lazy_t::identity();
+    auto slot_of = [&](uint32_t e) -> const g1_ed_slot_t* { return &bases[(e & 0x7fffffffu) & debug_idx_mask]; };
+    constexpr int A = SV_ED_AHEAD;
+    uint32_t e_q[A + 1];
+    g1_ed_operand_t raw_q[A];
+#pragma unroll
+    for (int i = 0; i <= A; i++) e_q[i] = lo + i < hi ? sorted[lo + i] : 0u;
+#pragma unroll
+    for (int i = 0; i < A; i++) raw_q[i] = g1_ed_operand_t::load(slot_of(e_q[i]));
+    for (uint32_t pos = lo;; pos++) {
+        const bool end = pos >= hi;
+        if (end || pos >= kend) {
+            acc.store_raw(&partial[start_k + part_off]);
+            if (end) break;
+            part_off = 0;
+            acc = ed_lazy_t::identity();
+            k++;
+            kend = kend2;
+            while (pos >= kend) {
+                k++;
+                kend = boff[k + 1];
+            }
+            kend2 = boff[k + 2 <= nbt ? k + 2 : nbt];
+            start_k = start[k];
+        }
+        const uint32_t e = e_q[0];
+        const g1_ed_operand_t raw = raw_q[0];
+#pragma unroll
+        for (int i = 0; i + 1 < A; i++) raw_q[i] = raw_q[i + 1];
+        if (pos + A < hi) raw_q[A - 1] = g1_ed_operand_t::load(slot_of(e_q[A]));
+#pragma unroll
+        for (int i = 0; i < A; i++) e_q[i] = e_q[i + 1];
+        if (pos + A + 1 < hi) e_q[A] = sorted[pos + A + 1];
+        fql_t ym, yp, kk;
+        raw.limbs(ym, yp, kk);
+        acc.madd(ym, yp, kk, (e >> 31) != 0);
+    }
+}
+static __global__ void __launch_bounds__(256) g1_ed_partials_to_xyzz_kernel(g1_lazy_partial_t* __restrict__ partial, const uint32_t* __restrict__ start,
+                                                                     uint32_t nbt) {
+    const uint32_t i = blockIdx.x * blockDim.x + threadIdx.x;
+    if (i >= start[nbt]) return;
+    ed_lazy_t::raw_to_xyzz(&partial[i]);
+}
+
 static __global__ void __launch_bounds__(256) g2_pair_partials_to_exact_kernel(const g2_pair_partial_t* __restrict__ raw, xyzz_mem_t<fq2_t>* __restrict__ partial,
                                                                         const uint32_t* __restrict__ start, uint32_t nbt) {
     const uint32_t g = blockIdx.x * blockDim.x + threadIdx.x;
diff --git a/snarkvm_amd/csrc/runtime.hip.h b/snarkvm_amd/csrc/runtime.hip.h
--- a/snarkvm_amd/csrc/runtime.hip.h
+++ b/snarkvm_amd/csrc/runtime.hip.h
@@ -378,6 +378,7 @@
     HIP_TRY(hipFuncSetAttribute((const void*)scan_one_block_kernel, hipFuncAttributeMaxDynamicSharedMemorySize, (int)(SCAN_ONE_MAX * 4)));
 #ifdef SV_TU_G1
     HIP_TRY(hipFuncSetAttribute((const void*)msm_accumulate_lazy_kernel<true>, hipFuncAttributeMaxDynamicSharedMemorySize, 128 * 1024));
+    HIP_TRY(hipFuncSetAttribute((const void*)msm_accumulate_ed_kernel<true>, hipFuncAttributeMaxDynamicSharedMemorySize, 128 * 1024));
 #endif
 #ifdef SV_TU_NTT
     HIP_TRY(hipFuncSetAttribute((const void*)ntt_pass_kernel_v2<false, ntt_arith_u>, hipFuncAttributeMaxDynamicSharedMemorySize, 96 * 1024));
@@ -635,6 +636,7 @@
     size_t n = 0;
     int tables = 1;
     int table_bits = 256;
+    int form = 0;
     mutable std::mutex co_mu;
     mutable std::condition_variable co_cv;
     mutable std::deque<msm_ticket_t*> co_q;
@@ -894,7 +896,7 @@
 }
 template <class F>
 static void msm_launch_accumulate(lane_t& c, const msm_plan_t& pl, const aff_mem_t<F>* vbase, uint32_t* boffp, uint32_t nbt, size_t nthreads, bool one_wave,
-                                  bool ltail) {
+                                  bool ltail, const aff_mem_t<F>* ed_origin = nullptr) {
     hipStream_t st = c.stream;
 #ifdef SV_BENCH
     static const uint32_t dbg_mask = getenv("SNARKVM_HIP_DEBUG_IDX_MASK") ? (uint32_t)strtoul(getenv("SNARKVM_HIP_DEBUG_IDX_MASK"), nullptr, 0) : 0xffffffffu;
@@ -906,8 +908,14 @@
         if (msm_lazy_on<F>()) {
             if (!ltail) c.part_raw.ensure(tmax * sizeof(g1_lazy_partial_t));
             g1_lazy_partial_t* raw_out = ltail ? c.part_a.as<g1_lazy_partial_t>() : c.part_raw.as<g1_lazy_partial_t>();
-            hipLaunchKernelGGL((msm_accumulate_lazy_kernel<true>), dim3((unsigned)((nthreads + 255) / 256)), dim3(256), one_wave || tuning().acc_one_wg ? msm_acc_lds() : 0, st,
-                               vbase, c.sorted.as<uint32_t>(), boffp, c.start_a.as<uint32_t>(), raw_out, nbt, pl.S, dbg_mask);
+            if (ed_origin) {
+                const g1_ed_slot_t* ed_base = (const g1_ed_slot_t*)ed_origin + (vbase - ed_origin);
+                hipLaunchKernelGGL((msm_accumulate_ed_kernel<true>), dim3((unsigned)((nthreads + 255) / 256)), dim3(256), one_wave || tuning().acc_one_wg ? msm_acc_lds() : 0,
+                                   st, ed_base, c.sorted.as<uint32_t>(), boffp, c.start_a.as<uint32_t>(), raw_out, nbt, pl.S, dbg_mask);
+                hipLaunchKernelGGL(g1_ed_partials_to_xyzz_kernel, dim3((unsigned)((tmax + 255) / 256)), dim3(256), 0, st, raw_out, (const uint32_t*)c.start_a.as<uint32_t>(), nbt);
+            } else
+                hipLaunchKernelGGL((msm_accumulate_lazy_kernel<true>), dim3((unsigned)((nthreads + 255) / 256)), dim3(256), one_wave || tuning().acc_one_wg ? msm_acc_lds() : 0, st,
+                                   vbase, c.sorted.as<uint32_t>(), boffp, c.start_a.as<uint32_t>(), raw_out, nbt, pl.S, dbg_mask);
             if (!ltail)
                 hipLaunchKernelGGL(g1_partials_to_exact_kernel, dim3((unsigned)((tmax + 255) / 256)), dim3(256), 0, st, (const g1_lazy_partial_t*)raw_out,
                                    c.part_a.as<g1_xyzz_mem_t>(), (const uint32_t*)c.start_a.as<uint32_t>(), nbt);
@@ -945,6 +953,8 @@
     int tables = 1;
     size_t table_stride = 0;
     int table_bits = 0;
+    int form = 0;
+    const aff_mem_t<F>* origin = nullptr;
     const uint4* scalars = nullptr;
     size_t n = 0;
     int scalars_montgomery = 0;
@@ -1231,7 +1241,8 @@
     if (mu && tuning().fuse_reduce < 0) rounds = mu->K >= 8 ? 1 : 0;
     hipLaunchKernelGGL(msm_alloc_seg_kernel, dim3((nbt + 1 + 255) / 256), dim3(256), 0, st, boffp, c.cnt_a.as<uint32_t>(), nbt, L.pl.S);
     exclusive_scan_u32(st, c.cnt_a.as<uint32_t>(), c.start_a.as<uint32_t>(), (size_t)nbt + 1, c.scan_tmp.as<uint32_t>());
-    msm_launch_accumulate<F>(c, L.pl, L.vbase, boffp, nbt, (L.E_max + L.pl.S - 1) / L.pl.S, L.single_round && L.prefetch_ok, L.ltail);
+    if (j.form && !(sizeof(F) == sizeof(fq_t) && msm_lazy_on<F>() && j.origin)) throw hip_failure{hipErrorInvalidValue, "msm: Edwards base slots need the lazy G1 accumulate kernel", __LINE__};
+    msm_launch_accumulate<F>(c, L.pl, L.vbase, boffp, nbt, (L.E_max + L.pl.S - 1) / L.pl.S, L.single_round && L.prefetch_ok, L.ltail, j.form ? j.origin : nullptr);
     ph.end();
     return rounds;
 }
@@ -1322,20 +1333,26 @@
 }
 #endif
 
+static int precompute_run_length(size_t n) {
+    const int run = (int)(n >> 16);
+    return run < 1 ? 1 : (run > PRE_RUN ? PRE_RUN : run);
+}
+template <class F>
+static void precompute_table_step(lane_t& c, const aff_mem_t<F>* prev, aff_mem_t<F>* next, size_t n, int table_bits) {
+    const int run = precompute_run_length(n);
+    const size_t slab = n < PRE_SLAB ? n : PRE_SLAB;
+    c.gen_pts.ensure(4 * slab * sizeof(typename F::mem_t));
+    for (size_t lo = 0; lo < n; lo += PRE_SLAB) {
+        const size_t cnt = n - lo < PRE_SLAB ? n - lo : PRE_SLAB;
+        const size_t threads = (cnt + run - 1) / run;
+        hipLaunchKernelGGL((precompute_table_kernel<F>), dim3((unsigned)((threads + 255) / 256)), dim3(256), 0, c.stream, prev + lo, next + lo, cnt, table_bits, run,
+                           (typename F::mem_t*)c.gen_pts.p);
+    }
+}
 template <class F>
 static void precompute_tables_run(lane_t& c, aff_mem_t<F>* d, size_t n, int tables, int table_bits) {
     if (tables <= 1 || !n) return;
-    int run = (int)(n >> 16);
-    run = run < 1 ? 1 : (run > PRE_RUN ? PRE_RUN : run);
-    const size_t slab = n < PRE_SLAB ? n : PRE_SLAB;
-    c.gen_pts.ensure(4 * slab * sizeof(typename F::mem_t));
-    for (int j = 1; j < tables; j++)
-        for (size_t lo = 0; lo < n; lo += PRE_SLAB) {
-            const size_t cnt = n - lo < PRE_SLAB ? n - lo : PRE_SLAB;
-            const size_t threads = (cnt + run - 1) / run;
-            hipLaunchKernelGGL((precompute_table_kernel<F>), dim3((unsigned)((threads + 255) / 256)), dim3(256), 0, c.stream, d + (size_t)(j - 1) * n + lo,
-                               d + (size_t)j * n + lo, cnt, table_bits, run, (typename F::mem_t*)c.gen_pts.p);
-        }
+    for (int j = 1; j < tables; j++) precompute_table_step<F>(c, d + (size_t)(j - 1) * n, d + (size_t)j * n, n, table_bits);
     HIP_TRY(hipGetLastError());
 }
 
@@ -1603,6 +1620,8 @@
     j.tables = h.tables;
     j.table_stride = h.n;
     j.table_bits = h.table_bits;
+    j.form = h.form;
+    j.origin = h.d[dev];
     j.n = r.n0 + r.n1;
     return j;
 }
diff --git a/snarkvm_amd/csrc/tuning.hip.h b/snarkvm_amd/csrc/tuning.hip.h
--- a/snarkvm_amd/csrc/tuning.hip.h
+++ b/snarkvm_amd/csrc/tuning.hip.h
@@ -6,7 +6,7 @@
 namespace sv {
 
 struct tuning_t {
-    int lazy = 1, lazy2 = 1, fused = 1;
+    int lazy = 1, lazy2 = 1, fused = 1, edwards = 1;
     long acc_lds = 96 * 1024;
     int acc_one_wg = 0, reduce_rounds = 1, fuse_batch = 1, fuse_max_k = 64, fuse_reduce = -1, coalesce = 1, coalesce_us = 40, lanes = 0;
     int msm_chunk_lg = 20, scalar_chunk_lg = 22, taper = 1, ring_lanes = 3, seg = 0, seg2 = 0, fold_l = 0, scan1 = 1;
@@ -19,7 +19,7 @@
         name = (decltype(name))v;          \
         return true;                       \
     }
-        SV_TUNE_KEY(lazy) SV_TUNE_KEY(lazy2) SV_TUNE_KEY(fused) SV_TUNE_KEY(acc_lds)
+        SV_TUNE_KEY(lazy) SV_TUNE_KEY(lazy2) SV_TUNE_KEY(fused) SV_TUNE_KEY(edwards) SV_TUNE_KEY(acc_lds)
         SV_TUNE_KEY(acc_one_wg) SV_TUNE_KEY(reduce_rounds) SV_TUNE_KEY(fuse_batch) SV_TUNE_KEY(fuse_max_k) SV_TUNE_KEY(fuse_reduce) SV_TUNE_KEY(coalesce)
         SV_TUNE_KEY(coalesce_us) SV_TUNE_KEY(lanes) SV_TUNE_KEY(msm_chunk_lg) SV_TUNE_KEY(scalar_chunk_lg) SV_TUNE_KEY(taper) SV_TUNE_KEY(ring_lanes) SV_TUNE_KEY(seg) SV_TUNE_KEY(seg2)
         SV_TUNE_KEY(fold_l) SV_TUNE_KEY(scan1) SV_TUNE_KEY(ntt_min_tiles) SV_TUNE_KEY(ntt_full_tw) SV_TUNE_KEY(ntt_fold)
diff --git a/snarkvm_amd/msm.py b/snarkvm_amd/msm.py
--- a/snarkvm_amd/msm.py
+++ b/snarkvm_amd/msm.py
@@ -44,6 +44,10 @@
         self.n = int(npoints)
         self._h = serialize.register_bases_serialized(data, npoints, compressed, validate, tables)
         return self
+
+    @property
+    def form(self):
+        return int(_lib.lib().snarkvm_hip_bases_form(self._h))
 
     def msm(self, scalars=None, offset=0, device_ptr=None, npoints=None, window_bits=0):
         L = _lib.lib()
```

Result: slower. 530.2 million pairs/s (-3.7%).
